# Chen001117/mappo

Measured on AMD Instinct MI355X. Metric: agent-steps/sec (collect+GAE+PPO), MPE simple_spread 3-agent, higher is better.
Workload: dtype f32; 1 GPU; BASELINE configs[1]: MPE simple_spread shape, 3 agents, obs 18 / share_obs 54 / Discrete(5), n_rollout_threads=1024 in total (strong scaling: 1024 on rank 0 of 1), episode_length=25, MLP policy (mappo), ppo_epoch=10, num_mini_batch=1, lr 7e-4, env=synthetic; n_rollout_threads_global=1024, n_rollout_threads_rank0=1024, episode_length=25, num_agents=3, ppo_epoch=10, num_mini_batch=1, parallelism=dp1, rccl_ranks=0, exact_minibatch_order=False, hip_graph=True

## Files before the change

### include/mappo_hip.h

```cpp
#ifndef MAPPO_HIP_H
#define MAPPO_HIP_H

#include <stdint.h>

#ifdef __cplusplus
extern "C" {
#endif

typedef void *mappo_stream_t;

#define MAPPO_OK 0
#define MAPPO_EINVAL (-1)
#define MAPPO_ELAUNCH (-2)
#define MAPPO_ENOTIMPL (-3)

#define MAPPO_HIDDEN 64
#define MAPPO_MAX_IN_DIM 512
#define MAPPO_MAX_ACTIONS 32
#define MAPPO_MAX_LAYER_N 2

const char *mappo_last_error(void);
int mappo_abi_version(void);

typedef struct {
// ... 19 lines not shown
                         float *rnn_dst, float *rnn_critic_dst, int32_t H, mappo_stream_t stream);

int mappo_insert_smac(const float *obs, const float *share_obs, const float *avail, const float *rewards, int64_t rew_stride_n,
                      int64_t rew_stride_m, const uint8_t *dones, int64_t done_stride_n, int64_t done_stride_m,
                      const uint8_t *bad_transition, const float *rnn_states, const float *rnn_states_critic, float *obs_dst,
                      float *share_dst, float *avail_dst, float *rew_dst, float *mask_dst, float *bad_mask_dst,
                      float *active_mask_dst, float *rnn_dst, float *rnn_critic_dst, int32_t N, int32_t M, int32_t D, int32_t S,
                      int32_t A, int32_t H, mappo_stream_t stream);

int mappo_recurrent_rows(const int64_t *perm, int32_t n_epochs, int64_t data_chunks, int32_t L, int32_t T, int32_t R,
                         int32_t num_mini_batch, int32_t *rows, int32_t *h0_rows, mappo_stream_t stream);

int mappo_copy_batch(int32_t count, float *const *dst, const float *const *src, const int64_t *n_floats, mappo_stream_t stream);

int mappo_gae_scan(const float *rewards , float *value_preds ,
                   const float *next_value , const float *masks ,
                   const float *bad_masks , float *returns ,
                   const float *vn_state , int32_t T, int32_t R, float gamma,
                   float gae_lambda, int32_t use_gae, int32_t use_proper_time_limits,
                   mappo_stream_t stream);

int64_t mappo_adv_workspace_bytes(int64_t n);
int mappo_adv_moments(const float *returns , const float *value_preds ,
                      const float *active_masks , const float *vn_state ,
                      float *adv , double *moments , void *workspace,
                      int64_t n, mappo_stream_t stream);
int mappo_adv_normalize(float *adv , const double *moments , int64_t n,
                        mappo_stream_t stream);

int64_t mappo_moments_workspace_bytes(int64_t B);
int mappo_minibatch_moments(const float *returns, const float *active_masks, const int32_t *rows,
                            int64_t B, double *mb_moments , void *workspace,
                            mappo_stream_t stream);
int mappo_valuenorm_update(float *vn_state , const double *mb_moments ,
                           double beta, mappo_stream_t stream);
int mappo_valuenorm_update_n(float *vn_state , const double *mb_moments , double beta, int32_t n,
                             float *states_out , mappo_stream_t stream);

typedef struct {
  float clip_param, entropy_coef, value_loss_coef, huber_delta;
  int32_t use_huber_loss, use_clipped_value_loss, use_policy_active_masks, use_value_active_masks,
      use_valuenorm;
  int32_t accumulate_partials;
} mappo_ppo_cfg;

int64_t mappo_ppo_loss_workspace_bytes(int64_t B);
int mappo_ppo_loss_fwd_bwd(const float *logits ,
                           const float *values , const int32_t *rows ,
                           const float *avail , const float *actions,
                           const float *old_logp, const float *adv, const float *active,
                           const float *v_old, const float *returns ,
                           const float *vn_state ,
                           const double *mb_moments ,
                           float *dlogits , float *dvalues , double *stats ,
                           void *workspace, const mappo_ppo_cfg *cfg , int64_t B, int32_t A,
                           mappo_stream_t stream);

int mappo_mlp_forward(const float *params, const mappo_net_desc *desc , const float *x ,
                      const int32_t *rows , int64_t B, float *out ,
                      mappo_stream_t stream);
int mappo_actor_act(const float *params, const mappo_net_desc *desc , const float *obs,
                    const float *avail , int64_t B, int32_t deterministic,
                    uint64_t seed, uint64_t counter, const uint64_t *counter_dev ,
                    float *actions , float *logp , mappo_stream_t stream);
int mappo_rollout_step(const float *actor_params, const mappo_net_desc *actor_desc , const float *critic_params,
                       const mappo_net_desc *critic_desc , const float *obs, int64_t obs_stride_n,
                       int64_t obs_stride_m, const float *share_obs, int64_t share_stride_n, int64_t share_stride_m,
                       int32_t M, int64_t B, const float *avail , int32_t deterministic, uint64_t seed,
                       uint64_t counter, const uint64_t *counter_dev, float *actions , float *logp ,
                       float *values , float *obs_dst , float *share_dst, const float *rewards,
                       int64_t rew_stride_n, int64_t rew_stride_m, const uint8_t *dones, int64_t done_stride_n,
                       int64_t done_stride_m, float *rew_dst, float *mask_dst, int32_t centralized, mappo_stream_t stream);
int mappo_actor_act_md(const float *params, const mappo_net_desc *desc , const float *obs, const float *avail ,
                       const int32_t *head_dims , int32_t n_heads, int64_t B, int32_t deterministic, uint64_t seed,
                       uint64_t counter, const uint64_t *counter_dev, float *actions , float *logp ,
                       mappo_stream_t stream);
int mappo_rollout_step_md(const float *actor_params, const mappo_net_desc *actor_desc , const float *critic_params,
                          const mappo_net_desc *critic_desc , const float *obs, int64_t obs_stride_n, int64_t obs_stride_m,
                          const float *share_obs, int64_t share_stride_n, int64_t share_stride_m, int32_t M, int64_t B,
                          const float *avail , const int32_t *head_dims , int32_t n_heads, int32_t deterministic,
                          uint64_t seed, uint64_t counter, const uint64_t *counter_dev, float *actions , float *logp ,
                          float *values , float *obs_dst , float *share_dst, const float *rewards,
                          int64_t rew_stride_n, int64_t rew_stride_m, const uint8_t *dones, int64_t done_stride_n, int64_t done_stride_m,
                          float *rew_dst, float *mask_dst, int32_t centralized, mappo_stream_t stream);
int mappo_rollout_episode(const float *actor_params, const mappo_net_desc *actor_desc , const float *critic_params,
                          const mappo_net_desc *critic_desc , int32_t T, int32_t N, int32_t M, const float *env_obs,
                          int64_t obs_stride_t, int64_t obs_stride_n, int64_t obs_stride_m, const float *rewards,
                          int64_t rew_stride_t, int64_t rew_stride_n, int64_t rew_stride_m, const uint8_t *dones,
                          int64_t done_stride_t, int64_t done_stride_n, int64_t done_stride_m, int32_t deterministic,
                          uint64_t seed, uint64_t counter, const uint64_t *counter_dev, float *obs_buf, float *share_buf,
                          float *rew_buf, float *mask_buf, float *actions , float *logp ,
                          float *values , float *next_values , int32_t centralized, mappo_stream_t stream);
int mappo_rollout_episode_uses_lds(int32_t layer_N);
int32_t mappo_mlp_backward_slabs(int64_t B);
int mappo_mlp_backward(const float *params, const mappo_net_desc *desc , const float *x,
                       const int32_t *rows, int64_t B, const float *dout ,
                       float *slabs, int64_t slab_stride, int64_t slab_col0,
                       float *wide_ws ,
                       mappo_stream_t stream);
#define MAPPO_WIDE_LAYOUT_FEATURE_MAJOR 0
#define MAPPO_WIDE_LAYOUT_BLOCKED 1
#define MAPPO_PRODUCER_MLP_BACKWARD 0
#define MAPPO_PRODUCER_ACTOR_UPDATE 1
#define MAPPO_PRODUCER_CRITIC_UPDATE 2
#define MAPPO_PRODUCER_TRUNK_BACKWARD 3
int64_t mappo_wide_workspace_floats(int64_t B);
int32_t mappo_wide_l1_slabs(int64_t B);
int32_t mappo_wide_layout(const mappo_net_desc *desc , int32_t producer );
int mappo_wide_l1_backward(const float *params, const mappo_net_desc *desc , const float *x, const int32_t *rows,
                           int64_t B, const float *wide_ws, float *slabs, int64_t slab_stride, int64_t slab_col0,
                           int32_t layout ,
                           mappo_stream_t stream);

int64_t mappo_update_partials_bytes(void);
int mappo_actor_update(const float *params, const mappo_net_desc *desc , const float *obs,
                       const int32_t *rows, int64_t B, const float *avail , const float *actions,
                       const float *old_logp, const float *adv, const float *active,
                       const double *mb_moments , const mappo_ppo_cfg *cfg , float *slabs,
                       int64_t slab_stride, int64_t slab_col0, double *partials, float *wide_ws ,
                       int32_t n_blocks ,
                       mappo_stream_t stream);
int mappo_critic_update(const float *params, const mappo_net_desc *desc , const float *share_obs,
                        const int32_t *rows, int64_t B, const float *v_old, const float *returns,
                        const float *active, const float *vn_state ,
                        const double *mb_moments , const mappo_ppo_cfg *cfg , float *slabs,
                        int64_t slab_stride, int64_t slab_col0, double *partials, float *wide_ws ,
                        int32_t n_blocks, mappo_stream_t stream);
int32_t mappo_dual_update_slabs(const mappo_net_desc *actor_desc , const mappo_net_desc *critic_desc , int64_t B);
int mappo_actor_critic_update(const float *actor_params, const mappo_net_desc *actor_desc , const float *obs,
                              const float *critic_params, const mappo_net_desc *critic_desc , const float *share_obs,
                              const int32_t *rows, int64_t B, const float *avail, const float *actions, const float *old_logp,
                              const float *adv, const float *active, const float *v_old, const float *returns,
                              const float *vn_state, const double *mb_moments, const mappo_ppo_cfg *cfg , float *slabs,
                              int64_t slab_stride, int64_t actor_col0, int64_t critic_col0, double *actor_partials,
                              double *critic_partials, mappo_stream_t stream);
int mappo_actor_update_md(const float *params, const mappo_net_desc *desc , const float *obs, const int32_t *rows, int64_t B,
                          const float *avail , const int32_t *head_dims , int32_t n_heads, const float *actions ,
                          const float *old_logp , const float *adv, const float *active, const double *mb_moments ,
                          const mappo_ppo_cfg *cfg , float *slabs, int64_t slab_stride, int64_t slab_col0, double *partials,
                          float *wide_ws , int32_t n_blocks, mappo_stream_t stream);
int mappo_actor_critic_update_md(const float *actor_params, const mappo_net_desc *actor_desc , const float *obs,
                                 const float *critic_params, const mappo_net_desc *critic_desc , const float *share_obs,
                                 const int32_t *rows, int64_t B, const float *avail , const int32_t *head_dims ,
                                 int32_t n_heads, const float *actions, const float *old_logp, const float *adv, const float *active,
                                 const float *v_old, const float *returns, const float *vn_state, const double *mb_moments,
                                 const mappo_ppo_cfg *cfg , float *slabs, int64_t slab_stride, int64_t actor_col0,
                                 int64_t critic_col0, double *actor_partials, double *critic_partials, mappo_stream_t stream);
int mappo_update_stats(const double *actor_partials, int32_t n_actor ,
                       const double *critic_partials, int32_t n_critic, const double *mb_moments,
                       const mappo_ppo_cfg *cfg , double *stats ,
                       double *acc ,
                       mappo_stream_t stream);

int mappo_mlp_features(const float *params, const mappo_net_desc *desc , const float *x, const int32_t *rows,
                       int64_t B, float *featT , mappo_stream_t stream);
int mappo_gru_forward(const float *params, const mappo_net_desc *desc , const float *featT, const float *h0,
                      const int32_t *h0_rows , const float *masks, const int32_t *rows ,
                      int32_t L, int32_t Nc, float *h_last ,
                      int32_t head_mode, float *out, const float *avail , int32_t deterministic,
                      uint64_t seed, uint64_t counter, const uint64_t *counter_dev, float *actions, float *logp,
                      mappo_stream_t stream);
int mappo_gru_step_dual(const float *actor_params, const mappo_net_desc *actor_desc , const float *actor_featT ,
                        const float *actor_h0 , float *actor_h_last, const float *critic_params,
                        const mappo_net_desc *critic_desc , const float *critic_featT, const float *critic_h0,
                        float *critic_h_last, const float *masks , int32_t Nc, const float *avail ,
                        int32_t deterministic, uint64_t seed, uint64_t counter, const uint64_t *counter_dev, float *actions,
                        float *logp, float *values, mappo_stream_t stream);
int mappo_recurrent_step_dual(const float *actor_params, const mappo_net_desc *actor_desc, const float *obs,
                              const float *actor_h0, float *actor_h_last, const float *critic_params,
                              const mappo_net_desc *critic_desc, const float *share_obs, const float *critic_h0,
                              float *critic_h_last, const float *masks, int32_t Nc, const float *avail, int32_t deterministic,
                              uint64_t seed, uint64_t counter, const uint64_t *counter_dev, float *actions, float *logp,
                              float *values, mappo_stream_t stream);
typedef struct mappo_smac_slot {
  float *obs, *share_obs, *available_actions , *rewards , *masks, *bad_masks, *active_masks, *rnn_states,
        *rnn_states_critic;
} mappo_smac_slot;
int mappo_recurrent_rollout_step(const float *actor_params, const mappo_net_desc *actor_desc , const float *critic_params,
                                 const mappo_net_desc *critic_desc , const float *obs, const float *share_obs, const float *avail,
                                 const float *rewards, int64_t rew_stride_n, int64_t rew_stride_m, const uint8_t *dones,
                                 int64_t done_stride_n, int64_t done_stride_m, const uint8_t *bad_transition ,
                                 const float *actor_h, const float *critic_h, float *actor_h_next, float *critic_h_next, int32_t N, int32_t M,
                                 int32_t deterministic, uint64_t seed, uint64_t counter, const uint64_t *counter_dev, float *actions,
                                 float *logp, float *values, const mappo_smac_slot *dst , mappo_stream_t stream);
int mappo_mlp_features_dual(const float *params_a, const mappo_net_desc *desc_a , const float *x_a, float *featT_a,
                            const float *params_c, const mappo_net_desc *desc_c , const float *x_c, float *featT_c,
                            int64_t B, mappo_stream_t stream);
int mappo_trunk_backward(const float *params, const mappo_net_desc *desc , const float *x, const int32_t *rows,
                         int64_t B, const float *dxT , float *slabs, int64_t slab_stride, int64_t slab_col0,
                         float *wide_ws , mappo_stream_t stream);

int64_t mappo_gru16_scratch_floats(int32_t L, int32_t Nc);
int64_t mappo_gru16_blocked_floats(int32_t L, int32_t Nc);
int32_t mappo_gru16_slabs(int32_t L, int32_t Nc);
int mappo_mlp_features_seq(const float *params, const mappo_net_desc *desc , const float *x, const int32_t *rows ,
                           int32_t L, int32_t Nc, float *out_blocked, mappo_stream_t stream);
int mappo_gru16_forward_loss(const float *params, const mappo_net_desc *desc , const float *x, int32_t x_blocked, const float *h0,
                             const int32_t *h0_rows , const float *masks, const int32_t *rows ,
                             int32_t L, int32_t Nc, int32_t head , const float *avail, const float *actions,
                             const float *old_logp, const float *adv, const float *active, const float *v_old, const float *returns,
                             const float *vn_state, const double *mb_moments, const mappo_ppo_cfg *cfg , float *scratch,
                             float *slabs, int64_t slab_stride, int64_t slab_col0, double *partials, mappo_stream_t stream);
int mappo_gru16_backward(const float *params, const mappo_net_desc *desc , const float *masks, const int32_t *rows, int32_t L,
                         int32_t Nc, float *scratch, float *dxT ,
                         mappo_stream_t stream);
int mappo_gru16_wgrad(const mappo_net_desc *desc , const float *x, int32_t x_blocked, const float *scratch, int32_t L, int32_t Nc,
                      float *slabs, int64_t slab_stride, int64_t slab_col0, mappo_stream_t stream);
int mappo_trunk_backward_seq(const float *params, const mappo_net_desc *desc , const float *x, const int32_t *rows, int32_t L,
                             int32_t Nc, const float *dx_blocked, float *slabs, int64_t slab_stride, int64_t slab_col0,
                             float *wide_ws ,
                             mappo_stream_t stream);

int64_t mappo_optim_workspace_bytes(int64_t P);
int mappo_slab_reduce(const float *slabs, int32_t n_slabs, int64_t slab_stride, int64_t P,
                      float *grad , mappo_stream_t stream);
int mappo_clip_adam(float *params, const float *grad, float *exp_avg, float *exp_avg_sq,
                    const int64_t *seg_bounds , int32_t n_seg,
                    const float *opt_hyper, int32_t *opt_step, float *grad_norms,
                    double *norm_acc , void *workspace,
                    mappo_stream_t stream);
int mappo_reduce_clip_adam(const float *slabs, int32_t n_slabs, int64_t slab_stride, float *params, float *grad ,
                           float *exp_avg, float *exp_avg_sq, const int64_t *seg_bounds , int32_t n_seg,
                           const float *opt_hyper, int32_t *opt_step, float *grad_norms, double *norm_acc ,
                           void *workspace, mappo_stream_t stream);

int mappo_mpe_spread_reset(double *agent_pos, double *agent_vel, double *landmark_pos, int32_t *tstep, int64_t *episode, float *obs,
                           int32_t N, int32_t M, int32_t L, uint64_t seed, mappo_stream_t stream);
int mappo_mpe_spread_step(double *agent_pos, double *agent_vel, double *landmark_pos, int32_t *tstep, int64_t *episode,
                          const float *actions, int32_t action_mode, float *obs, float *rewards, uint8_t *dones, int32_t N, int32_t M,
                          int32_t L, int32_t episode_length, uint64_t seed, mappo_stream_t stream);
int mappo_rollout_episode_spread(const float *actor_params, const mappo_net_desc *actor_desc , const float *critic_params,
                                 const mappo_net_desc *critic_desc , int32_t T, int32_t N, int32_t M, int32_t L,
                                 int32_t env_episode_length, uint64_t env_seed, double *agent_pos, double *agent_vel,
                                 double *landmark_pos, int32_t *tstep, int64_t *episode, int32_t deterministic, uint64_t seed,
                                 uint64_t counter, const uint64_t *counter_dev, float *obs_buf, float *share_buf, float *rew_buf,
                                 float *mask_buf, float *actions , float *logp , float *values ,
                                 float *next_values , int32_t centralized, mappo_stream_t stream);

int mappo_mpe_reference_reset(double *agent_pos, double *agent_vel, double *landmark_pos, int32_t *goal, int32_t *tstep,
                              int64_t *episode, float *obs, int32_t N, uint64_t seed, mappo_stream_t stream);
int mappo_mpe_reference_step(double *agent_pos, double *agent_vel, double *landmark_pos, int32_t *goal, int32_t *tstep,
                             int64_t *episode, const float *actions, int32_t action_mode, float *obs, float *rewards, uint8_t *dones,
                             int32_t N, int32_t episode_length, uint64_t seed, mappo_stream_t stream);
int mappo_rollout_episode_reference(const float *actor_params, const mappo_net_desc *actor_desc , const float *critic_params,
                                    const mappo_net_desc *critic_desc , const int32_t *head_dims ,
                                    int32_t n_heads, int32_t T, int32_t N, int32_t env_episode_length, uint64_t env_seed,
                                    double *agent_pos, double *agent_vel, double *landmark_pos, int32_t *goal, int32_t *tstep,
                                    int64_t *episode, int32_t deterministic, uint64_t seed, uint64_t counter,
                                    const uint64_t *counter_dev, float *obs_buf, float *share_buf, float *rew_buf, float *mask_buf,
                                    float *actions , float *logp , float *values ,
                                    float *next_values , int32_t centralized, mappo_stream_t stream);

int mappo_mpe_comm_reset(double *listener_pos, double *listener_vel, double *landmark_pos, int32_t *goal, int32_t *symbol,
                         int32_t *tstep, int64_t *episode, float *obs_speaker, float *obs_listener, int32_t N, uint64_t seed,
                         mappo_stream_t stream);
int mappo_mpe_comm_step(double *listener_pos, double *listener_vel, double *landmark_pos, int32_t *goal, int32_t *symbol,
                        int32_t *tstep, int64_t *episode, const float *actions_speaker, const float *actions_listener,
                        int32_t action_mode, float *obs_speaker, float *obs_listener, float *rewards, uint8_t *dones, int32_t N,
                        int32_t episode_length, uint64_t seed, mappo_stream_t stream);
typedef struct mappo_comm_agent {
  const float *actor_params, *critic_params;
  mappo_net_desc actor_desc, critic_desc;
  uint64_t seed;
  const uint64_t *counter_dev;
  float *obs_buf, *share_buf, *rew_buf, *mask_buf, *actions, *logp, *values, *next_values;
} mappo_comm_agent;
int mappo_rollout_episode_comm(const mappo_comm_agent *speaker , const mappo_comm_agent *listener , int32_t T,
                               int32_t N, int32_t env_episode_length, uint64_t env_seed, double *listener_pos, double *listener_vel,
                               double *landmark_pos, int32_t *goal, int32_t *symbol, int32_t *tstep, int64_t *episode,
                               int32_t deterministic, uint64_t counter, int32_t centralized,
                               mappo_stream_t stream);

int mappo_mpe_adversary_reset(double *agent_pos, double *agent_vel, double *landmark_pos, int32_t *goal, int32_t *tstep,
                              int64_t *episode, float *obs_adversary, float *obs_good1, float *obs_good2, int32_t N,
                              int32_t num_agents, uint64_t seed, mappo_stream_t stream);
int mappo_mpe_adversary_step(double *agent_pos, double *agent_vel, double *landmark_pos, int32_t *goal, int32_t *tstep,
                             int64_t *episode, const float *actions, int32_t action_mode, float *obs_adversary, float *obs_good1,
                             float *obs_good2, float *rewards, uint8_t *dones, int32_t N, int32_t num_agents,
                             int32_t episode_length, uint64_t seed, mappo_stream_t stream);
int mappo_rollout_episode_adversary(const mappo_comm_agent *agents , double *agent_pos, double *agent_vel,
                                    double *landmark_pos, int32_t *goal, int32_t *tstep, int64_t *episode, int32_t T, int32_t N,
                                    int32_t env_episode_length, uint64_t env_seed, int32_t deterministic, uint64_t counter,
                                    int32_t centralized, mappo_stream_t stream);

int mappo_synth_smac_pool(float *obs, float *share_obs, float *avail, float *rewards, uint8_t *dead, uint8_t *dones, int32_t P,
                          int32_t N, int32_t M, int32_t D, int32_t S, int32_t A, float p_death, float p_term, uint64_t seed,
                          uint64_t *counter_dev , mappo_stream_t stream);
int mappo_synth_smac_step(float *obs, float *share_obs, float *avail, float *rewards, uint8_t *dead, uint8_t *dones,
                          int32_t N, int32_t M, int32_t D, int32_t S, int32_t A, float p_death, float p_term,
                          uint64_t seed, uint64_t *counter_dev , mappo_stream_t stream);

#define MAPPO_PROF_GAE 0
#define MAPPO_PROF_PPO_LOSS 1
#define MAPPO_PROF_MLP_FWD 2
#define MAPPO_PROF_MLP_BWD 3
#define MAPPO_PROF_SLAB_REDUCE 4
#define MAPPO_PROF_ADAM 5
#define MAPPO_PROF_ACT 6
#define MAPPO_PROF_COUNT 8
int mappo_profile_arm(int32_t kernel_id, void *ev_start , void *ev_stop );

int mappo_selftest_mfma(const float *A , const float *Bm , float *D ,
                        mappo_stream_t stream);

#ifdef __cplusplus
}
// ... 3 lines not shown
```

### mappo_amd/_lib.py

```python
import ctypes as C
import os

import torch

_HERE = os.path.dirname(os.path.abspath(__file__))
LIB_PATH = os.environ.get("MAPPO_HIP_LIB") or os.path.join(_HERE, "libmappo_hip.so")

HIDDEN = 64
MAX_ACTIONS = 32
MAX_LAYER_N = 2


class NetDesc(C.Structure):
    _fields_ = [("in_dim", C.c_int32), ("hidden", C.c_int32), ("out_dim", C.c_int32), ("layer_N", C.c_int32),
                ("use_relu", C.c_int32), ("use_feature_norm", C.c_int32), ("recurrent", C.c_int32)]


class PpoCfg(C.Structure):
    _fields_ = [("clip_param", C.c_float), ("entropy_coef", C.c_float), ("value_loss_coef", C.c_float),
                ("huber_delta", C.c_float), ("use_huber_loss", C.c_int32), ("use_clipped_value_loss", C.c_int32),
                ("use_policy_active_masks", C.c_int32), ("use_value_active_masks", C.c_int32),
                ("use_valuenorm", C.c_int32), ("accumulate_partials", C.c_int32)]


class SmacSlot(C.Structure):
    _fields_ = [(n, C.c_void_p) for n in ("obs", "share_obs", "available_actions", "rewards", "masks", "bad_masks", "active_masks",
                                          "rnn_states", "rnn_states_critic")]


class CommAgent(C.Structure):
    _fields_ = ([("actor_params", C.c_void_p), ("critic_params", C.c_void_p), ("actor_desc", NetDesc), ("critic_desc", NetDesc),
                 ("seed", C.c_uint64), ("counter_dev", C.c_void_p)] +
                [(n, C.c_void_p) for n in ("obs_buf", "share_buf", "rew_buf", "mask_buf", "actions", "logp", "values", "next_values")])


_P, _I32, _I64, _F, _D, _U64 = C.c_void_p, C.c_int32, C.c_int64, C.c_float, C.c_double, C.c_uint64

SIGNATURES = {
    "mappo_last_error": (C.c_char_p, []),
    "mappo_abi_version": (C.c_int, []),
    "mappo_net_param_count": (_I64, [C.POINTER(NetDesc)]),
    "mappo_insert_mpe": (C.c_int, [_P, _I64, _I64, _P, _I64, _I64, _P, _I64, _I64, _P, _P, _P, _P, _I32, _I32, _I32, _I32, _P]),
    "mappo_insert_mpe_rnn": (C.c_int, [_P, _I64, _I64, _P, _I64, _I64, _P, _I64, _I64, _P, _P, _P, _P, _I32, _I32, _I32, _I32, _P, _P, _P, _P,
                                       _I32, _P]),
    "mappo_insert_smac": (C.c_int, [_P, _P, _P, _P, _I64, _I64, _P, _I64, _I64, _P, _P, _P] + [_P] * 9 + [_I32] * 6 + [_P]),
    "mappo_recurrent_rows": (C.c_int, [_P, _I32, _I64, _I32, _I32, _I32, _I32, _P, _P, _P]),
    "mappo_copy_batch": (C.c_int, [_I32, C.POINTER(C.c_void_p), C.POINTER(C.c_void_p), C.POINTER(_I64), _P]),
    "mappo_gae_scan": (C.c_int, [_P, _P, _P, _P, _P, _P, _P, _I32, _I32, _F, _F, _I32, _I32, _P]),
    "mappo_adv_workspace_bytes": (_I64, [_I64]),
    "mappo_adv_moments": (C.c_int, [_P, _P, _P, _P, _P, _P, _P, _I64, _P]),
    "mappo_adv_normalize": (C.c_int, [_P, _P, _I64, _P]),
    "mappo_moments_workspace_bytes": (_I64, [_I64]),
    "mappo_minibatch_moments": (C.c_int, [_P, _P, _P, _I64, _P, _P, _P]),
    "mappo_valuenorm_update": (C.c_int, [_P, _P, _D, _P]),
    "mappo_valuenorm_update_n": (C.c_int, [_P, _P, _D, _I32, _P, _P]),
    "mappo_ppo_loss_workspace_bytes": (_I64, [_I64]),
    "mappo_ppo_loss_fwd_bwd": (C.c_int, [_P] * 16 + [C.POINTER(PpoCfg), _I64, _I32, _P]),
    "mappo_mlp_forward": (C.c_int, [_P, C.POINTER(NetDesc), _P, _P, _I64, _P, _P]),
    "mappo_actor_act": (C.c_int, [_P, C.POINTER(NetDesc), _P, _P, _I64, _I32, _U64, _U64, _P, _P, _P, _P]),
    "mappo_rollout_step": (C.c_int, [_P, C.POINTER(NetDesc), _P, C.POINTER(NetDesc), _P, _I64, _I64, _P, _I64, _I64, _I32, _I64, _P, _I32,
                                     _U64, _U64, _P, _P, _P, _P, _P, _P, _P, _I64, _I64, _P, _I64, _I64, _P, _P, _I32, _P]),
    "mappo_actor_act_md": (C.c_int, [_P, C.POINTER(NetDesc), _P, _P, C.POINTER(_I32), _I32, _I64, _I32, _U64, _U64, _P, _P, _P, _P]),
    "mappo_rollout_step_md": (C.c_int, [_P, C.POINTER(NetDesc), _P, C.POINTER(NetDesc), _P, _I64, _I64, _P, _I64, _I64, _I32, _I64, _P,
                                        C.POINTER(_I32), _I32, _I32, _U64, _U64, _P, _P, _P, _P, _P, _P, _P, _I64, _I64, _P, _I64, _I64, _P, _P,
                                        _I32, _P]),
    "mappo_rollout_episode": (C.c_int, [_P, C.POINTER(NetDesc), _P, C.POINTER(NetDesc), _I32, _I32, _I32, _P, _I64, _I64, _I64, _P, _I64,
                                        _I64, _I64, _P, _I64, _I64, _I64, _I32, _U64, _U64, _P, _P, _P, _P, _P, _P, _P, _P, _P, _I32, _P]),
    "mappo_rollout_episode_uses_lds": (C.c_int, [_I32]),
    "mappo_mlp_backward_slabs": (_I32, [_I64]),
    "mappo_mlp_backward": (C.c_int, [_P, C.POINTER(NetDesc), _P, _P, _I64, _P, _P, _I64, _I64, _P, _P]),
    "mappo_wide_workspace_floats": (_I64, [_I64]),
    "mappo_wide_l1_slabs": (_I32, [_I64]),
    "mappo_wide_layout": (_I32, [C.POINTER(NetDesc), _I32]),
    "mappo_wide_l1_backward": (C.c_int, [_P, C.POINTER(NetDesc), _P, _P, _I64, _P, _P, _I64, _I64, _I32, _P]),
    "mappo_update_partials_bytes": (_I64, []),
    "mappo_actor_update": (C.c_int, [_P, C.POINTER(NetDesc), _P, _P, _I64, _P, _P, _P, _P, _P, _P, C.POINTER(PpoCfg), _P, _I64,
                                     _I64, _P, _P, _I32, _P]),
    "mappo_critic_update": (C.c_int, [_P, C.POINTER(NetDesc), _P, _P, _I64, _P, _P, _P, _P, _P, C.POINTER(PpoCfg), _P, _I64,
                                      _I64, _P, _P, _I32, _P]),
    "mappo_dual_update_slabs": (_I32, [C.POINTER(NetDesc), C.POINTER(NetDesc), _I64]),
    "mappo_actor_critic_update": (C.c_int, [_P, C.POINTER(NetDesc), _P, _P, C.POINTER(NetDesc), _P, _P, _I64, _P, _P, _P, _P, _P, _P, _P, _P, _P,
                                            C.POINTER(PpoCfg), _P, _I64, _I64, _I64, _P, _P, _P]),
    "mappo_actor_update_md": (C.c_int, [_P, C.POINTER(NetDesc), _P, _P, _I64, _P, C.POINTER(_I32), _I32, _P, _P, _P, _P, _P, C.POINTER(PpoCfg),
                                        _P, _I64, _I64, _P, _P, _I32, _P]),
    "mappo_actor_critic_update_md": (C.c_int, [_P, C.POINTER(NetDesc), _P, _P, C.POINTER(NetDesc), _P, _P, _I64, _P, C.POINTER(_I32), _I32,
                                               _P, _P, _P, _P, _P, _P, _P, _P, C.POINTER(PpoCfg), _P, _I64, _I64, _I64, _P, _P, _P]),
    "mappo_update_stats": (C.c_int, [_P, _I32, _P, _I32, _P, C.POINTER(PpoCfg), _P, _P, _P]),
    "mappo_mlp_features": (C.c_int, [_P, C.POINTER(NetDesc), _P, _P, _I64, _P, _P]),
    "mappo_gru_forward": (C.c_int, [_P, C.POINTER(NetDesc), _P, _P, _P, _P, _P, _I32, _I32, _P, _I32, _P, _P, _I32, _U64, _U64,
                                    _P, _P, _P, _P]),
    "mappo_gru_step_dual": (C.c_int, [_P, C.POINTER(NetDesc), _P, _P, _P, _P, C.POINTER(NetDesc), _P, _P, _P, _P, _I32, _P, _I32, _U64, _U64,
                                      _P, _P, _P, _P, _P]),
    "mappo_recurrent_step_dual": (C.c_int, [_P, C.POINTER(NetDesc), _P, _P, _P, _P, C.POINTER(NetDesc), _P, _P, _P, _P, _I32, _P, _I32, _U64, _U64,
                                      _P, _P, _P, _P, _P]),
    "mappo_gru16_scratch_floats": (_I64, [_I32, _I32]),
    "mappo_gru16_blocked_floats": (_I64, [_I32, _I32]),
    "mappo_gru16_slabs": (_I32, [_I32, _I32]),
    "mappo_mlp_features_seq": (C.c_int, [_P, C.POINTER(NetDesc), _P, _P, _I32, _I32, _P, _P]),
    "mappo_gru16_forward_loss": (C.c_int, [_P, C.POINTER(NetDesc), _P, _I32, _P, _P, _P, _P, _I32, _I32, _I32] + [_P] * 9 +
                                 [C.POINTER(PpoCfg), _P, _P, _I64, _I64, _P, _P]),
    "mappo_gru16_backward": (C.c_int, [_P, C.POINTER(NetDesc), _P, _P, _I32, _I32, _P, _P, _P]),
    "mappo_gru16_wgrad": (C.c_int, [C.POINTER(NetDesc), _P, _I32, _P, _I32, _I32, _P, _I64, _I64, _P]),
    "mappo_trunk_backward_seq": (C.c_int, [_P, C.POINTER(NetDesc), _P, _P, _I32, _I32, _P, _P, _I64, _I64, _P, _P]),
    "mappo_recurrent_rollout_step": (C.c_int, [_P, C.POINTER(NetDesc), _P, C.POINTER(NetDesc), _P, _P, _P, _P, _I64, _I64, _P, _I64, _I64, _P,
                                               _P, _P, _P, _P, _I32, _I32, _I32, _U64, _U64, _P, _P, _P, _P, C.POINTER(SmacSlot), _P]),
    "mappo_mlp_features_dual": (C.c_int, [_P, C.POINTER(NetDesc), _P, _P, _P, C.POINTER(NetDesc), _P, _P, _I64, _P]),
    "mappo_trunk_backward": (C.c_int, [_P, C.POINTER(NetDesc), _P, _P, _I64, _P, _P, _I64, _I64, _P, _P]),
    "mappo_optim_workspace_bytes": (_I64, [_I64]),
    "mappo_slab_reduce": (C.c_int, [_P, _I32, _I64, _I64, _P, _P]),
    "mappo_clip_adam": (C.c_int, [_P, _P, _P, _P, C.POINTER(_I64), _I32, _P, _P, _P, _P, _P, _P]),
    "mappo_reduce_clip_adam": (C.c_int, [_P, _I32, _I64, _P, _P, _P, _P, C.POINTER(_I64), _I32, _P, _P, _P, _P, _P, _P]),
    "mappo_mpe_spread_reset": (C.c_int, [_P, _P, _P, _P, _P, _P, _I32, _I32, _I32, _U64, _P]),
    "mappo_synth_smac_pool": (C.c_int, [_P, _P, _P, _P, _P, _P, _I32, _I32, _I32, _I32, _I32, _I32, C.c_float, C.c_float, _U64, _P, _P]),
    "mappo_synth_smac_step": (C.c_int, [_P, _P, _P, _P, _P, _P, _I32, _I32, _I32, _I32, _I32, C.c_float, C.c_float, _U64, _P, _P]),
    "mappo_mpe_spread_step": (C.c_int, [_P, _P, _P, _P, _P, _P, _I32, _P, _P, _P, _I32, _I32, _I32, _I32, _U64, _P]),
    "mappo_rollout_episode_spread": (C.c_int, [_P, C.POINTER(NetDesc), _P, C.POINTER(NetDesc), _I32, _I32, _I32, _I32, _I32, _U64, _P, _P, _P, _P,
                                               _P, _I32, _U64, _U64, _P, _P, _P, _P, _P, _P, _P, _P, _P, _I32, _P]),
    "mappo_mpe_reference_reset": (C.c_int, [_P, _P, _P, _P, _P, _P, _P, _I32, _U64, _P]),
    "mappo_mpe_reference_step": (C.c_int, [_P, _P, _P, _P, _P, _P, _P, _I32, _P, _P, _P, _I32, _I32, _U64, _P]),
    "mappo_rollout_episode_reference": (C.c_int, [_P, C.POINTER(NetDesc), _P, C.POINTER(NetDesc), C.POINTER(_I32), _I32, _I32, _I32, _I32, _U64,
                                                  _P, _P, _P, _P, _P, _P, _I32, _U64, _U64, _P, _P, _P, _P, _P, _P, _P, _P, _P, _I32, _P]),
    "mappo_mpe_comm_reset": (C.c_int, [_P, _P, _P, _P, _P, _P, _P, _P, _P, _I32, _U64, _P]),
    "mappo_mpe_comm_step": (C.c_int, [_P, _P, _P, _P, _P, _P, _P, _P, _P, _I32, _P, _P, _P, _P, _I32, _I32, _U64, _P]),
    "mappo_rollout_episode_comm": (C.c_int, [C.POINTER(CommAgent), C.POINTER(CommAgent), _I32, _I32, _I32, _U64, _P, _P, _P, _P, _P, _P, _P,
                                             _I32, _U64, _I32, _P]),
    "mappo_mpe_adversary_reset": (C.c_int, [_P, _P, _P, _P, _P, _P, _P, _P, _P, _I32, _I32, _U64, _P]),
    "mappo_mpe_adversary_step": (C.c_int, [_P, _P, _P, _P, _P, _P, _P, _I32, _P, _P, _P, _P, _P, _I32, _I32, _I32, _U64, _P]),
    "mappo_rollout_episode_adversary": (C.c_int, [C.POINTER(CommAgent), _P, _P, _P, _P, _P, _P, _I32, _I32, _I32, _U64, _I32, _U64, _I32, _P]),
    "mappo_profile_arm": (C.c_int, [_I32, _P, _P]),
    "mappo_selftest_mfma": (C.c_int, [_P, _P, _P, _P]),
}

_lib = None


class MappoHipError(RuntimeError):
    pass


def load():
    global _lib
    if _lib is not None:
        return _lib
    if not os.path.exists(LIB_PATH):
        raise MappoHipError(f"{LIB_PATH} is missing — build it with `python -m mappo_amd.build` "
                            "(hipcc --offload-arch=gfx950).  There is no CPU fallback for the MAPPO hot path.")
    lib = C.CDLL(LIB_PATH)
    for name, (res, args) in SIGNATURES.items():
        fn = getattr(lib, name)
        fn.restype, fn.argtypes = res, args
    _lib = lib
    return lib


def check(rc, what):
    if rc != 0:
        msg = load().mappo_last_error().decode("utf-8", "replace")
        raise MappoHipError(f"{what} failed (code {rc}): {msg}")
```

### mappo_amd/algorithms/r_mappo/r_mappo.py

```python
import numpy as np
import os
import torch

from mappo_amd import ops
from mappo_amd.utils.util import to_device_f32
from mappo_amd.utils.valuenorm import ValueNorm


class R_MAPPO():
    def __init__(self, args, policy, device=torch.device("cuda"), dist_group=None):
        self.device = torch.device(device)
        self.tpdv = dict(dtype=torch.float32, device=self.device)
        self.policy = policy
        self.args = args

        self.clip_param = args.clip_param
        self.ppo_epoch = args.ppo_epoch
        self.num_mini_batch = args.num_mini_batch
        self.data_chunk_length = args.data_chunk_length
        self.value_loss_coef = args.value_loss_coef
        self.entropy_coef = args.entropy_coef
        self.max_grad_norm = args.max_grad_norm
        self.huber_delta = args.huber_delta

        self._use_recurrent_policy = args.use_recurrent_policy
        self._use_naive_recurrent = args.use_naive_recurrent_policy
        self._use_max_grad_norm = args.use_max_grad_norm
        self._use_clipped_value_loss = args.use_clipped_value_loss
        self._use_huber_loss = args.use_huber_loss
        self._use_popart = args.use_popart
        self._use_valuenorm = args.use_valuenorm
        self._use_value_active_masks = args.use_value_active_masks
        self._use_policy_active_masks = args.use_policy_active_masks
        self._exact_order = bool(getattr(args, "exact_minibatch_order", False))
        self._fused = not bool(getattr(args, "unfused_update", False))
        self._use_graph = bool(getattr(args, "use_hip_graph", True))
        self._concurrent_update = bool(getattr(args, "concurrent_update", False))
        self._graphs = {}
        self._dp_graphs = {}
        self._graph_buffers = {}

        assert (self._use_popart and self._use_valuenorm) == False, \
            "self._use_popart and self._use_valuenorm can not be set True simultaneously"
        if self._use_popart:
            raise NotImplementedError("use_popart: PopArt.update raises in the reference itself (SURVEY.md §8c)")
        self.value_normalizer = ValueNorm(1, device=self.device) if self._use_valuenorm else None

        self._cfg = ops.ppo_cfg(args)
        self._cfg_acc = ops.ppo_cfg(args, accumulate_partials=True)
        self._dual_update = bool(getattr(args, "dual_update", True)) and os.environ.get("MAPPO_DUAL_UPDATE", "1") != "0"
        self._epochs = None
        self._dist = dist_group
        if getattr(policy.actor, "head_dims", None):
            if dist_group is not None:
                raise NotImplementedError("MultiDiscrete action space under the data-parallel trainer: the multi-head update is built for "
                                          "single-process training only")
            if not self._fused:
                raise NotImplementedError("unfused_update with a MultiDiscrete action space: the loss of several heads exists in the fused "
                                          "update kernels only")
        if dist_group is not None:
            from mappo_amd.distributed import sampling_seed
            policy.actor._seed = sampling_seed(int(getattr(args, "seed", 1)), dist_group.rank)
        f64 = dict(dtype=torch.float64, device=self.device)
        self._mb_moments = torch.zeros(4, **f64)
        self._adv_moments = torch.zeros(3, **f64)
        self._stats = torch.zeros(6, **f64)
        self._zbuf = torch.zeros(8 + 2 * 1024, **f64)
        self._acc = self._zbuf[:6]
        self._pa, self._pc = self._zbuf[8:8 + 1024], self._zbuf[8 + 1024:]
        self._ws = {}
        self._training = False

    def _buf(self, name, shape, dtype=torch.float32, zero=False):
        key = (name, tuple(shape), dtype)
        t = self._ws.get(key)
        if t is None:
            t = (torch.zeros if zero else torch.empty)(shape, dtype=dtype, device=self.device)
            self._ws[key] = t
        return t

    def _bytes(self, name, nbytes):
        return self._buf(name, (int(nbytes),), torch.uint8)

    def _update(self, src, rows, B, update_actor=True, moments_ready=False, part="all"):
        pol = self.policy
        A = pol.actor.n_actions
        lib = ops._lib.load()
        vn_state = self.value_normalizer.state if self._use_valuenorm else None
        n_slabs = ops.mlp_backward_slabs(B)
        P = pol.n_flat
        if part != "optim":
            self._slab_rows = n_slabs
            slabs = self._update_kernels(src, rows, B, update_actor, moments_ready, vn_state, n_slabs, P)
            n_slabs = self._slab_rows
        else:
            slabs = self._buf("slabs", (n_slabs, P))
        if update_actor != self._actor_enabled and part != "kernels":
            pol.opt_hyper[0, 7] = 1.0 if update_actor else 0.0
            self._actor_enabled = update_actor
        if self._dist is None:
            ops.reduce_clip_adam(slabs, n_slabs, P, pol.flat_params, pol.flat_grad, pol.exp_avg, pol.exp_avg_sq, pol.seg_bounds,
                                 pol.opt_hyper, pol.opt_step, pol.grad_norms, pol.opt_workspace, norm_acc=self._acc[4:])
            return
        if part != "optim":
            ops.slab_reduce(slabs, n_slabs, P, P, pol.flat_grad)
        if part != "kernels":
            self._dist.all_reduce_sum_(pol.flat_grad)
            ops.clip_adam(pol.flat_params, pol.flat_grad, pol.exp_avg, pol.exp_avg_sq, pol.seg_bounds, pol.opt_hyper,
                          pol.opt_step, pol.grad_norms, pol.opt_workspace, norm_acc=self._acc[4:])

    def _moments(self, src, rows, B, vn_state):
        lib = ops._lib.load()
        ops.minibatch_moments(src["returns"], src["active"], rows, B, self._mb_moments,
                              self._bytes("mom_ws", lib.mappo_moments_workspace_bytes(B)))
        if self._dist is not None:
            self._dist.all_reduce_sum_(self._mb_moments)
        ep = self._epochs
        if ep is not None and self._use_valuenorm:
            ops.valuenorm_update_n(vn_state, self._mb_moments, self.value_normalizer.beta, ep["n"], ep["states"])

    def _update_kernels(self, src, rows, B, update_actor, moments_ready, vn_state, n_slabs, P):
        pol = self.policy
        A = pol.actor.n_actions
        lib = ops._lib.load()
        ep = self._epochs
        if not moments_ready:
            self._moments(src, rows, B, vn_state)
        cfg = self._cfg
        if ep is not None:
            cfg = self._cfg_acc
            if self._use_valuenorm:
                vn_state = ep["states"][ep["e"]]
        elif self._use_valuenorm:
            ops.valuenorm_update(vn_state, self._mb_moments, self.value_normalizer.beta)
        hd = pol.actor.head_dims
        slabs = self._buf("slabs", (n_slabs, P), zero=True)
        if not update_actor and not self._actor_slabs_clean:
            slabs[:, :pol.seg_bounds[1]].zero_()
        self._actor_slabs_clean = not update_actor
        if self._fused:
            pa, pc = self._pa, self._pc
            na, nc = (0, 0)
            if update_actor and self._concurrent_update and not hd:
                na, nc = self._split_grid(n_slabs, pol.actor.desc.in_dim, pol.critic.desc.in_dim, B)
            if na:
                cur = torch.cuda.current_stream()
                if self._side_stream is None:
                    self._side_stream = torch.cuda.Stream(device=self.device)
                side = self._side_stream
                side.wait_stream(cur)
                with torch.cuda.stream(side):
                    ops.actor_update(pol.actor.flat, pol.actor.desc, src["obs"], rows, B, src["avail"], src["actions"],
                                     src["old_logp"], src["adv"], src["active"], self._mb_moments, cfg, slabs, P, 0, pa, na)
                ops.critic_update(pol.critic.flat, pol.critic.desc, src["share_obs"], rows, B, src["v_old"], src["returns"],
                                  src["active"], vn_state, self._mb_moments, cfg, slabs, P, pol.seg_bounds[1], pc, nc)
                cur.wait_stream(side)
                n_pa, n_pc = na, nc
            elif hd and update_actor and self._dual_update and pol.can_dual_update():
                ops.actor_critic_update_md(pol.actor.flat, pol.actor.desc, src["obs"], pol.critic.flat, pol.critic.desc, src["share_obs"],
                                           rows, B, hd, src["actions"], src["old_logp"], src["adv"], src["active"], src["v_old"],
                                           src["returns"], vn_state, self._mb_moments, cfg, slabs, P, 0, pol.seg_bounds[1], pa, pc)
                n_pa = n_pc = ops.dual_update_slabs(pol.actor.desc, pol.critic.desc, B)
                self._slab_rows = n_pa
            elif update_actor and self._dual_update and pol.can_dual_update():
                ops.actor_critic_update(pol.actor.flat, pol.actor.desc, src["obs"], pol.critic.flat, pol.critic.desc, src["share_obs"],
                                        rows, B, src["avail"], src["actions"], src["old_logp"], src["adv"], src["active"], src["v_old"],
                                        src["returns"], vn_state, self._mb_moments, cfg, slabs, P, 0, pol.seg_bounds[1], pa, pc)
                n_pa = n_pc = ops.dual_update_slabs(pol.actor.desc, pol.critic.desc, B)
                self._slab_rows = n_pa
            else:
                if update_actor and hd:
                    ops.actor_update_md(pol.actor.flat, pol.actor.desc, src["obs"], rows, B, hd, src["actions"], src["old_logp"],
                                        src["adv"], src["active"], self._mb_moments, cfg, slabs, P, 0, pa)
                elif update_actor:
                    ops.actor_update(pol.actor.flat, pol.actor.desc, src["obs"], rows, B, src["avail"], src["actions"],
                                     src["old_logp"], src["adv"], src["active"], self._mb_moments, cfg, slabs, P, 0, pa)
                ops.critic_update(pol.critic.flat, pol.critic.desc, src["share_obs"], rows, B, src["v_old"], src["returns"],
                                  src["active"], vn_state, self._mb_moments, cfg, slabs, P, pol.seg_bounds[1], pc)
                n_pa = n_pc = n_slabs
            if ep is None:
                ops.update_stats(pa if update_actor else None, n_pa, pc, n_pc, self._mb_moments, self._cfg, self._stats, self._acc)

        else:
            logits = self._buf("logits", (B, A))
            values = self._buf("values", (B,))
            ops.mlp_forward(pol.actor.flat, pol.actor.desc, src["obs"], rows, B, logits)
            ops.mlp_forward(pol.critic.flat, pol.critic.desc, src["share_obs"], rows, B, values)
            dlogits = self._buf("dlogits", (B, A))
            dvalues = self._buf("dvalues", (B,))
            ops.ppo_loss_fwd_bwd(logits, values, rows, src["avail"], src["actions"], src["old_logp"], src["adv"],
                                 src["active"], src["v_old"], src["returns"], vn_state, self._mb_moments, dlogits, dvalues,
                                 self._stats, self._cfg, self._bytes("loss_ws", lib.mappo_ppo_loss_workspace_bytes(B)))
            self._acc[:4].add_(self._stats[:4])
            if update_actor:
                ops.mlp_backward(pol.actor.flat, pol.actor.desc, src["obs"], rows, B, dlogits, slabs, P, 0)
            ops.mlp_backward(pol.critic.flat, pol.critic.desc, src["share_obs"], rows, B, dvalues, slabs, P, pol.seg_bounds[1])
        return slabs

    _actor_slabs_clean = True
    _actor_enabled = True
    _side_stream = None

    @staticmethod
    def _split_grid(n_slabs, d_actor, d_critic, B):
        if n_slabs < 256 or d_actor > 64 or d_critic > 64:
            return 0, 0
        tiles = (B + 31) // 32
        cost = lambda d: 1.0 + 0.25 * (d > 32)
        best = None
        for na in range(96, 161, 4):
            nc = 256 - na
            t = max(-(-tiles // (4 * na)) * cost(d_actor), -(-tiles // (4 * nc)) * cost(d_critic))
            if best is None or t < best[0]:
                best = (t, na, nc)
        return best[1], best[2]

    def _buffer_sources(self, buffer, adv):
        T = buffer.episode_length
        R = buffer.n_rollout_threads * buffer.num_agents
        S = T * R
        flat = lambda a: a[:T].view(S, -1)
        return dict(obs=flat(buffer.obs), share_obs=flat(buffer.share_obs),
                    avail=flat(buffer.available_actions) if buffer.available_actions is not None else None,
                    actions=buffer.actions.view(S, -1).squeeze(-1), old_logp=buffer.action_log_probs.view(S, -1).squeeze(-1), adv=adv,
                    active=buffer.active_masks[:T].view(S), v_old=buffer.value_preds[:T].view(S),
                    returns=buffer.returns[:T].view(S)), S

    @torch.no_grad()
    def train(self, buffer, update_actor=True, after_update=False):
        self._sync_actor_mode(update_actor)
        if self._use_recurrent_policy or self._use_naive_recurrent:
            from mappo_amd.recurrent import train_recurrent
            static = buffer.perm_device != "cpu"
            body = lambda: (train_recurrent(self, buffer, update_actor), buffer.after_update() if after_update else None)
        else:
            static = self.num_mini_batch == 1 and not self._exact_order
            body = lambda: self._train_body(buffer, update_actor, after_update)
        if not (self._use_graph and static and self._dist is None):
            body()
            return self._finish_train_info()
        key = (self._buffer_key(buffer), bool(update_actor), bool(after_update))
        state = self._graphs.get(key)
        if state is None:
            body()
            self._graphs[key] = "warm"
        else:
            if state == "warm":
                torch.cuda.synchronize()
                g = torch.cuda.CUDAGraph()
                with torch.cuda.graph(g):
                    body()
                self._graphs[key] = state = g
            state.replay()
        return self._finish_train_info()

    def _buffer_key(self, buffer):
        k = id(buffer)
        held = self._graph_buffers.setdefault(k, buffer)
        assert held is buffer
        return k

    def _sync_actor_mode(self, update_actor):
        if update_actor != self._actor_enabled:
            self.policy.opt_hyper[0, 7] = 1.0 if update_actor else 0.0
            self._actor_enabled = update_actor
        if not update_actor and not self._actor_slabs_clean:
            for (name, _, _), t in self._ws.items():
                if name == "slabs" or name.startswith("slabs_rec/"):
                    t[:, :self.policy.seg_bounds[1]].zero_()
        self._actor_slabs_clean = not update_actor

    def _train_body(self, buffer, update_actor, after_update):
        T = buffer.episode_length
        S = T * buffer.n_rollout_threads * buffer.num_agents
        adv = self.compute_advantages(buffer)
        src, _ = self._buffer_sources(buffer, adv)
        self._zbuf.zero_()
        whole = self.num_mini_batch == 1 and not self._exact_order
        dp_graph = self._dist is not None and self._use_graph and whole and self._fused and self._dist.world_is_gpu
        key = (self._buffer_key(buffer), bool(update_actor))
        self._epochs = None
        if whole and self._fused and (self._dist is None or dp_graph) and not self._concurrent_update \
                and os.environ.get("MAPPO_EPOCH_BATCH", "1") != "0":
            self._epochs = dict(n=self.ppo_epoch, e=0, states=self._buf("vn_states", (self.ppo_epoch, 3)))
        if dp_graph:
            vn_state = self.value_normalizer.state if self._use_valuenorm else None
            self._moments(src, None, S, vn_state)
        for epoch in range(self.ppo_epoch):
            if self._epochs is not None:
                self._epochs["e"] = epoch
            if whole:
                batches = [(None, S)]
            else:
                batches = [(rows, rows.numel()) for rows in buffer.feed_forward_rows(self.num_mini_batch)]
            for rows, B in batches:
                if dp_graph:
                    gkey = key + (epoch,)
                    st = self._dp_graphs.get(gkey)
                    if st is None and self._dp_graphs.get(key) == "warm":
                        st = "warm"
                    if st == "warm":
                        torch.cuda.synchronize()
                        try:
                            g = torch.cuda.CUDAGraph()
                            with torch.cuda.graph(g, capture_error_mode="thread_local"):
                                self._update(src, rows, B, update_actor, moments_ready=True, part="kernels")
                            self._dp_graphs[gkey] = st = g
                        except Exception as e:
                            import warnings
                            warnings.warn(f"hipGraph capture of the data-parallel update segment failed ({e}); launching eagerly")
                            torch.cuda.synchronize()
                            self._dp_graphs[gkey] = st = "off"
                    if st == "off":
                        st = None
                    if st is None:
                        self._update(src, rows, B, update_actor, moments_ready=True, part="kernels")
                    else:
                        st.replay()
                    self._update(src, rows, B, update_actor, moments_ready=True, part="optim")
                else:
                    self._update(src, rows, B, update_actor, moments_ready=whole and epoch > 0)
        if self._epochs is not None:
            n_rows = ops.dual_update_slabs(self.policy.actor.desc, self.policy.critic.desc, S) if (update_actor and self._dual_update and self.policy.can_dual_update()) \
                else ops.mlp_backward_slabs(S)
            ops.update_stats(self._pa if update_actor else None, n_rows, self._pc, n_rows, self._mb_moments, self._cfg, self._stats,
                             self._acc)
            self._epochs = None
        if dp_graph and self._dp_graphs.get(key) is None:
            self._dp_graphs[key] = "warm"
        if after_update:
            buffer.after_update()

    def compute_advantages(self, buffer):
        T = buffer.episode_length
        S = T * buffer.n_rollout_threads * buffer.num_agents
        adv = self._buf("adv", (S,))
        lib = ops._lib.load()
        vn_state = self.value_normalizer.state if self._use_valuenorm else None
        ops.adv_moments(buffer.returns[:T].view(S), buffer.value_preds[:T].view(S), buffer.active_masks[:T].view(S), vn_state,
                        adv, self._adv_moments, self._bytes("adv_ws", lib.mappo_adv_workspace_bytes(S)))
        if self._dist is not None:
            self._dist.all_reduce_sum_(self._adv_moments)
        ops.adv_normalize(adv, self._adv_moments)
        return adv

    def _finish_train_info(self):
        num_updates = self.ppo_epoch * self.num_mini_batch
        if self._dist is not None:
            self._dist.all_reduce_sum_(self._acc[:4])
        acc = (self._acc / max(num_updates, 1)).cpu().numpy()
        return dict(value_loss=float(acc[0]), policy_loss=float(acc[1]), dist_entropy=float(acc[2]),
                    actor_grad_norm=float(acc[4]), critic_grad_norm=float(acc[5]), ratio=float(acc[3]))

    @torch.no_grad()
    def ppo_update(self, sample, update_actor=True):
        if self._use_recurrent_policy or self._use_naive_recurrent:
            from mappo_amd.recurrent import ppo_update_recurrent
            return ppo_update_recurrent(self, sample, update_actor)
        (share_obs, obs, rnn_a, rnn_c, actions, v_old, ret, masks, active, old_logp, adv, avail) = sample
        d = lambda x: to_device_f32(x, self.device)
        B = np.shape(obs)[0] if not torch.is_tensor(obs) else obs.shape[0]
        src = dict(obs=d(obs), share_obs=d(share_obs), avail=d(avail) if avail is not None else None,
                   actions=d(actions).view(B, -1).squeeze(-1), old_logp=d(old_logp).view(B, -1).squeeze(-1), adv=d(adv).view(B),
                   active=d(active).view(B),
                   v_old=d(v_old).view(B), returns=d(ret).view(B))
        self._acc.zero_()
        self._update(src, None, B, update_actor)
        a = self._acc.cpu().numpy()
        return a[0], a[5], a[1], a[2], a[4], a[3]

    @torch.no_grad()
    def cal_value_loss(self, values, value_preds_batch, return_batch, active_masks_batch):
        d = lambda x: to_device_f32(x, self.device)
        values, value_preds_batch, return_batch, active_masks_batch = d(values), d(value_preds_batch), d(return_batch), d(active_masks_batch)
        clipped = value_preds_batch + (values - value_preds_batch).clamp(-self.clip_param, self.clip_param)
        if self._use_valuenorm:
            self.value_normalizer.update(return_batch)
            tgt = self.value_normalizer.normalize(return_batch)
        else:
            tgt = return_batch
        e_c, e_o = tgt - clipped, tgt - values

        def loss(e):
            if self._use_huber_loss:
                dl = self.huber_delta
                return torch.where(e.abs() <= dl, e * e / 2, dl * (e.abs() - dl / 2))
            return e * e / 2
        l = torch.max(loss(e_o), loss(e_c)) if self._use_clipped_value_loss else loss(e_o)
        if self._use_value_active_masks:
            return (l * active_masks_batch).sum() / active_masks_batch.sum()
        return l.mean()

    def prep_training(self):
        self._training = True

    def prep_rollout(self):
        self._training = False
```

### mappo_amd/config.py

```python
import argparse


def get_config():
    p = argparse.ArgumentParser(description="mappo_amd", formatter_class=argparse.RawDescriptionHelpFormatter)
    off = dict(action="store_false", default=True)
    on = dict(action="store_true", default=False)
    p.add_argument("--algorithm_name", type=str, default="mappo", choices=["rmappo", "mappo"])
    p.add_argument("--experiment_name", type=str, default="check")
    p.add_argument("--seed", type=int, default=1)
    p.add_argument("--cuda", **off)
    p.add_argument("--cuda_deterministic", **off)
    p.add_argument("--n_training_threads", type=int, default=1)
    p.add_argument("--n_rollout_threads", type=int, default=32)
    p.add_argument("--n_eval_rollout_threads", type=int, default=1)
    p.add_argument("--n_render_rollout_threads", type=int, default=1)
    p.add_argument("--num_env_steps", type=int, default=10e6)
    p.add_argument("--user_name", type=str, default="marl")
    p.add_argument("--use_wandb", **off)
    p.add_argument("--env_name", type=str, default="StarCraft2")
    p.add_argument("--use_obs_instead_of_state", **on)
    p.add_argument("--episode_length", type=int, default=200)
    p.add_argument("--share_policy", **off)
    p.add_argument("--use_centralized_V", **off)
    p.add_argument("--stacked_frames", type=int, default=1)
    p.add_argument("--use_stacked_frames", **on)
    p.add_argument("--hidden_size", type=int, default=64)
    p.add_argument("--layer_N", type=int, default=1)
    p.add_argument("--use_ReLU", **off)
    p.add_argument("--use_popart", **on)
    p.add_argument("--use_valuenorm", **off)
    p.add_argument("--use_feature_normalization", **off)
    p.add_argument("--use_orthogonal", **off)
    p.add_argument("--gain", type=float, default=0.01)
    p.add_argument("--use_naive_recurrent_policy", **on)
    p.add_argument("--use_recurrent_policy", **off)
    p.add_argument("--recurrent_N", type=int, default=1)
    p.add_argument("--data_chunk_length", type=int, default=10)
    p.add_argument("--lr", type=float, default=5e-4)
    p.add_argument("--critic_lr", type=float, default=5e-4)
    p.add_argument("--opti_eps", type=float, default=1e-5)
    p.add_argument("--weight_decay", type=float, default=0)
    p.add_argument("--ppo_epoch", type=int, default=15)
    p.add_argument("--use_clipped_value_loss", **off)
    p.add_argument("--clip_param", type=float, default=0.2)
    p.add_argument("--num_mini_batch", type=int, default=1)
    p.add_argument("--entropy_coef", type=float, default=0.01)
    p.add_argument("--value_loss_coef", type=float, default=1)
    p.add_argument("--use_max_grad_norm", **off)
    p.add_argument("--max_grad_norm", type=float, default=10.0)
    p.add_argument("--use_gae", **off)
    p.add_argument("--gamma", type=float, default=0.99)
    p.add_argument("--gae_lambda", type=float, default=0.95)
    p.add_argument("--use_proper_time_limits", **on)
    p.add_argument("--use_huber_loss", **off)
    p.add_argument("--use_value_active_masks", **off)
    p.add_argument("--use_policy_active_masks", **off)
    p.add_argument("--huber_delta", type=float, default=10.0)
    p.add_argument("--use_linear_lr_decay", **on)
    p.add_argument("--save_interval", type=int, default=1)
    p.add_argument("--log_interval", type=int, default=5)
    p.add_argument("--use_eval", **on)
    p.add_argument("--eval_interval", type=int, default=25)
    p.add_argument("--eval_episodes", type=int, default=32)
    p.add_argument("--save_gifs", **on)
    p.add_argument("--use_render", **on)
    p.add_argument("--render_episodes", type=int, default=5)
    p.add_argument("--ifi", type=float, default=0.1)
    p.add_argument("--model_dir", type=str, default=None)
    p.add_argument("--exact_minibatch_order", **on,
                   help="with num_mini_batch == 1 the minibatch is the whole buffer and its permutation only reorders "
                        "the terms of sums; by default the kernels then stream the buffer in place. Set to gather by "
                        "the random permutation anyway (what the reference's generator does).")
    p.add_argument("--unfused_update", **on,
                   help="run each PPO update as separate forward / fused-loss / backward launches (the standalone C-ABI ops) "
                        "instead of the one-launch-per-network update kernels; same results")
    p.add_argument("--use_hip_graph", **off,
                   help="by default the launch-bound inner loops (PPO updates; rollout with a graph-safe env) are captured "
                        "into hipGraphs after one eager pass; pass the flag to always launch eagerly")
    p.add_argument("--host_staging", **off,
                   help="by default the NumPy output of a CPU vec-env goes through pinned double-buffered staging blocks "
                        "(mappo_amd/utils/host_staging.py) and feeds the same one-launch rollout step as a device env; pass the "
                        "flag to upload with plain torch copies")
    p.add_argument("--fuse_rollout_step", **off,
                   help="by default an MLP policy's rollout step (insert of the previous env output + get_actions + get_values) "
                        "is ONE kernel launch (mappo_rollout_step); pass the flag to use the separate insert / actor / critic launches")
    p.add_argument("--fuse_rollout_episode", **off,
                   help="by default, with an env that hands out a whole episode up front (SyntheticMPEEnv.episode_block) and a "
                        "narrow MLP policy, the rollout episode (T x get_actions, T + 1 x get_values, every insert) is ONE kernel "
                        "launch (mappo_rollout_episode); with the GPU-resident simple_spread env (SimpleSpreadVecEnv.episode_state) the env "
                        "steps run inside that launch too (mappo_rollout_episode_spread), and so they do with the GPU-resident simple_reference env "
                        "and its MultiDiscrete (5, 10) policy (SimpleReferenceVecEnv, mappo_rollout_episode_reference); pass the flag to run "
                        "the stepwise loop")
    p.add_argument("--dual_update", **off,
                   help="by default the actor's and the critic's fused update run in ONE launch, half the CUs each "
                        "(mappo_actor_critic_update); pass the flag to launch them one after the other")
    p.add_argument("--concurrent_update", **on,
                   help="launch the actor and critic update kernels side by side on a split grid (two streams); measured "
                        "slower than back-to-back full-size launches on MI355X, kept for experiments")
    p.add_argument("--perm_device", type=str, default="cuda", choices=["cuda", "cpu"],
                   help="where torch.randperm runs; 'cpu' reproduces the reference's permutation stream bit-exactly")
    return p


def mpe_defaults(parser):
    parser.add_argument("--scenario_name", type=str, default="simple_spread",
                        help="MPE scenario; GPU-resident envs exist for simple_spread, simple_reference, simple_speaker_listener "
                             "(num_agents 2, share_policy False) and simple_adversary (num_agents 3, share_policy False): mappo_amd.envs")
    parser.add_argument("--num_landmarks", type=int, default=3)
    parser.add_argument("--num_agents", type=int, default=2)
    return parser


def apply_algorithm_name(all_args):
    if all_args.algorithm_name == "rmappo":
        all_args.use_recurrent_policy, all_args.use_naive_recurrent_policy = True, False
    elif all_args.algorithm_name == "mappo":
        all_args.use_recurrent_policy, all_args.use_naive_recurrent_policy = False, False
    else:
        raise NotImplementedError(all_args.algorithm_name)
    return all_args
```

### mappo_amd/csrc/error.hip

```cpp
#include "common.h"
#include <string.h>

static thread_local char g_err[512] = "";

void mappo_set_error(const char *fmt, ...) {
  va_list ap;
  va_start(ap, fmt);
  vsnprintf(g_err, sizeof(g_err), fmt, ap);
  va_end(ap);
}

extern "C" const char *mappo_last_error(void) { return g_err; }
extern "C" int mappo_abi_version(void) { return 7; }

ProfSlot g_prof[MAPPO_PROF_COUNT] = {};

extern "C" int mappo_profile_arm(int32_t kernel_id, void *ev_start, void *ev_stop) {
  MAPPO_REQUIRE(kernel_id >= 0 && kernel_id < MAPPO_PROF_COUNT, "profile_arm: kernel_id %d", kernel_id);
  g_prof[kernel_id].start = (hipEvent_t)ev_start;
  g_prof[kernel_id].stop = (hipEvent_t)ev_stop;
  return MAPPO_OK;
}
```

### mappo_amd/csrc/insert.hip

```cpp
#include "insert_core.h"

__global__ __launch_bounds__(256) void insert_mpe_kernel(InsertArgs p) { insert_mpe_body(p, blockIdx.x, gridDim.x); }

extern "C" int mappo_insert_mpe(const float *obs, int64_t obs_stride_n, int64_t obs_stride_m, const float *rewards,
                                int64_t rew_stride_n, int64_t rew_stride_m, const uint8_t *dones, int64_t done_stride_n,
                                int64_t done_stride_m, float *obs_dst, float *share_dst, float *rew_dst, float *mask_dst,
                                int32_t N, int32_t M, int32_t D, int32_t centralized, mappo_stream_t stream) {
  MAPPO_REQUIRE(obs && rewards && dones && obs_dst && share_dst && rew_dst && mask_dst && N > 0 && M > 0 && D > 0,
                "insert_mpe: bad arguments");
  InsertArgs a;
  a.obs = obs; a.obs_sn = obs_stride_n; a.obs_sm = obs_stride_m; a.rew = rewards; a.rew_sn = rew_stride_n; a.rew_sm = rew_stride_m;
  a.done = dones; a.done_sn = done_stride_n; a.done_sm = done_stride_m; a.obs_dst = obs_dst; a.share_dst = share_dst;
  a.rew_dst = rew_dst; a.mask_dst = mask_dst; a.N = N; a.M = M; a.D = D; a.centralized = centralized;
  const int64_t total = (int64_t)N * M * (centralized ? M * D : D);
  int64_t nb = (total + 255) / 256;
  if (nb > 2048) nb = 2048;
  hipLaunchKernelGGL(insert_mpe_kernel, dim3((unsigned)nb), dim3(256), 0, as_stream(stream), a);
  MAPPO_CHECK_LAUNCH("insert_mpe");
  return MAPPO_OK;
}

struct RnnInsert {
  const float *h_a, *h_c;
  float *dst_a, *dst_c;
  int H;
};
__global__ __launch_bounds__(256) void insert_mpe_rnn_kernel(InsertArgs p, RnnInsert r) {
  insert_mpe_body(p, blockIdx.x, gridDim.x);
  const int h4 = r.H >> 2;
  const int64_t total = (int64_t)p.N * p.M * h4;
  for (int64_t e = (int64_t)blockIdx.x * blockDim.x + threadIdx.x; e < total; e += (int64_t)gridDim.x * blockDim.x) {
    const int64_t nm = e / h4;
    const int n = (int)(nm / p.M), m = (int)(nm - (int64_t)n * p.M);
    const float keep = p.done[n * p.done_sn + m * p.done_sm] ? 0.f : 1.f;
    float4 a = reinterpret_cast<const float4 *>(r.h_a)[e], c = reinterpret_cast<const float4 *>(r.h_c)[e];
    a.x *= keep; a.y *= keep; a.z *= keep; a.w *= keep;
    c.x *= keep; c.y *= keep; c.z *= keep; c.w *= keep;
    reinterpret_cast<float4 *>(r.dst_a)[e] = a;
    reinterpret_cast<float4 *>(r.dst_c)[e] = c;
  }
}

extern "C" int mappo_insert_mpe_rnn(const float *obs, int64_t obs_stride_n, int64_t obs_stride_m, const float *rewards,
                                    int64_t rew_stride_n, int64_t rew_stride_m, const uint8_t *dones, int64_t done_stride_n,
                                    int64_t done_stride_m, float *obs_dst, float *share_dst, float *rew_dst, float *mask_dst,
                                    int32_t N, int32_t M, int32_t D, int32_t centralized, const float *rnn_states,
                                    const float *rnn_states_critic, float *rnn_dst, float *rnn_critic_dst, int32_t H,
                                    mappo_stream_t stream) {
  MAPPO_REQUIRE(obs && rewards && dones && obs_dst && share_dst && rew_dst && mask_dst && N > 0 && M > 0 && D > 0,
                "insert_mpe_rnn: bad arguments");
  MAPPO_REQUIRE(rnn_states && rnn_states_critic && rnn_dst && rnn_critic_dst && H > 0 && (H & 3) == 0, "insert_mpe_rnn: bad state arguments");
  MAPPO_REQUIRE(((((uintptr_t)rnn_states) | ((uintptr_t)rnn_states_critic) | ((uintptr_t)rnn_dst) | ((uintptr_t)rnn_critic_dst)) & 15) == 0,
                "insert_mpe_rnn: state arrays must be 16-byte aligned");
  InsertArgs a;
  a.obs = obs; a.obs_sn = obs_stride_n; a.obs_sm = obs_stride_m; a.rew = rewards; a.rew_sn = rew_stride_n; a.rew_sm = rew_stride_m;
  a.done = dones; a.done_sn = done_stride_n; a.done_sm = done_stride_m; a.obs_dst = obs_dst; a.share_dst = share_dst;
  a.rew_dst = rew_dst; a.mask_dst = mask_dst; a.N = N; a.M = M; a.D = D; a.centralized = centralized;
  RnnInsert r;
  r.h_a = rnn_states; r.h_c = rnn_states_critic; r.dst_a = rnn_dst; r.dst_c = rnn_critic_dst; r.H = H;
  const int64_t t1 = (int64_t)N * M * (centralized ? M * D : D), t2 = (int64_t)N * M * (H >> 2);
  int64_t nb = ((t1 > t2 ? t1 : t2) + 255) / 256;
  if (nb > 2048) nb = 2048;
  hipLaunchKernelGGL(insert_mpe_rnn_kernel, dim3((unsigned)nb), dim3(256), 0, as_stream(stream), a, r);
  MAPPO_CHECK_LAUNCH("insert_mpe_rnn");
  return MAPPO_OK;
}

__global__ __launch_bounds__(256) void insert_smac_kernel(SmacInsert p) { insert_smac_body(p, blockIdx.x, gridDim.x); }

extern "C" int mappo_insert_smac(const float *obs, const float *share_obs, const float *avail, const float *rewards, int64_t rew_stride_n,
                                 int64_t rew_stride_m, const uint8_t *dones, int64_t done_stride_n, int64_t done_stride_m,
                                 const uint8_t *bad_transition, const float *rnn_states, const float *rnn_states_critic, float *obs_dst,
                                 float *share_dst, float *avail_dst, float *rew_dst, float *mask_dst, float *bad_mask_dst,
                                 float *active_mask_dst, float *rnn_dst, float *rnn_critic_dst, int32_t N, int32_t M, int32_t D,
                                 int32_t S, int32_t A, int32_t H, mappo_stream_t stream) {
  MAPPO_REQUIRE(obs && share_obs && rewards && dones && obs_dst && share_dst && rew_dst && mask_dst && bad_mask_dst && active_mask_dst &&
                N > 0 && M > 0 && D > 0 && S > 0, "insert_smac: bad arguments");
  MAPPO_REQUIRE(!avail || (avail_dst && A > 0), "insert_smac: available_actions slot");
  if (rnn_states) {
    MAPPO_REQUIRE(rnn_states_critic && rnn_dst && rnn_critic_dst && H > 0 && (H & 3) == 0, "insert_smac: bad state arguments");
    MAPPO_REQUIRE(((((uintptr_t)rnn_states) | ((uintptr_t)rnn_states_critic) | ((uintptr_t)rnn_dst) | ((uintptr_t)rnn_critic_dst)) & 15) == 0,
                  "insert_smac: state arrays must be 16-byte aligned");
  }
  SmacInsert a;
  a.obs = obs; a.share = share_obs; a.avail = avail; a.rew = rewards; a.rew_sn = rew_stride_n; a.rew_sm = rew_stride_m;
  a.done = dones; a.done_sn = done_stride_n; a.done_sm = done_stride_m; a.bad = bad_transition; a.h_a = rnn_states; a.h_c = rnn_states_critic;
  a.obs_dst = obs_dst; a.share_dst = share_dst; a.avail_dst = avail_dst; a.rew_dst = rew_dst; a.mask_dst = mask_dst; a.bad_dst = bad_mask_dst;
  a.active_dst = active_mask_dst; a.ha_dst = rnn_dst; a.hc_dst = rnn_critic_dst; a.N = N; a.M = M; a.D = D; a.S = S; a.A = A; a.H = H;
  int64_t most = (int64_t)N * M * (D > S ? D : S);
  int64_t nb = (most + 255) / 256;
  if (nb > 2048) nb = 2048;
  hipLaunchKernelGGL(insert_smac_kernel, dim3((unsigned)nb), dim3(256), 0, as_stream(stream), a);
  MAPPO_CHECK_LAUNCH("insert_smac");
  return MAPPO_OK;
}

struct RecRows {
  const int64_t *perm;
  int32_t *rows, *h0;
  int64_t chunks;
  int E, L, T, R, nmb, mbs;
};
__global__ __launch_bounds__(256) void recurrent_rows_kernel(RecRows p) {
  const int64_t per_e = (int64_t)p.nmb * p.mbs, total = (int64_t)p.E * per_e * p.L;
  for (int64_t i = (int64_t)blockIdx.x * blockDim.x + threadIdx.x; i < total; i += (int64_t)gridDim.x * blockDim.x) {
    const int64_t j = i % p.mbs;
    const int l = (int)((i / p.mbs) % p.L);
    const int64_t ek = i / ((int64_t)p.mbs * p.L);
    const int64_t e = ek / p.nmb, k = ek - e * p.nmb;
    const int64_t c = p.perm[e * p.chunks + k * p.mbs + j];
    const int64_t q = c * p.L + l;
    const int32_t row = (int32_t)((q % p.T) * p.R + q / p.T);
    p.rows[i] = row;
    if (l == 0) p.h0[ek * p.mbs + j] = row;
  }
}

extern "C" int mappo_recurrent_rows(const int64_t *perm, int32_t n_epochs, int64_t data_chunks, int32_t L, int32_t T, int32_t R,
                                    int32_t num_mini_batch, int32_t *rows, int32_t *h0_rows, mappo_stream_t stream) {
  MAPPO_REQUIRE(perm && rows && h0_rows && n_epochs > 0 && data_chunks > 0 && L > 0 && T > 0 && R > 0 && num_mini_batch > 0,
                "recurrent_rows: bad arguments");
  MAPPO_REQUIRE(data_chunks / num_mini_batch > 0, "recurrent_rows: fewer chunks than minibatches");
  MAPPO_REQUIRE((int64_t)T * R < ((int64_t)1 << 31), "recurrent_rows: buffer rows exceed int32");
  RecRows a;
  a.perm = perm; a.rows = rows; a.h0 = h0_rows; a.chunks = data_chunks; a.E = n_epochs; a.L = L; a.T = T; a.R = R;
  a.nmb = num_mini_batch; a.mbs = (int)(data_chunks / num_mini_batch);
  const int64_t total = (int64_t)n_epochs * a.nmb * a.mbs * L;
  int64_t nb = (total + 255) / 256;
  if (nb > 4096) nb = 4096;
  hipLaunchKernelGGL(recurrent_rows_kernel, dim3((unsigned)nb), dim3(256), 0, as_stream(stream), a);
  MAPPO_CHECK_LAUNCH("recurrent_rows");
  return MAPPO_OK;
}

#define COPY_MAX 16
struct CopyBatch {
  float *dst[COPY_MAX];
  const float *src[COPY_MAX];
  int64_t n[COPY_MAX];
  int count;
};
__global__ __launch_bounds__(256) void copy_batch_kernel(CopyBatch c) {
  for (int j = 0; j < c.count; ++j) {
    const float *__restrict__ s = c.src[j];
    float *__restrict__ d = c.dst[j];
    const int64_t n = c.n[j];
    if (((((uintptr_t)s) | ((uintptr_t)d)) & 15) == 0) {
      const int64_t n4 = n >> 2;
      for (int64_t i = (int64_t)blockIdx.x * blockDim.x + threadIdx.x; i < n4; i += (int64_t)gridDim.x * blockDim.x)
        reinterpret_cast<float4 *>(d)[i] = reinterpret_cast<const float4 *>(s)[i];
      for (int64_t i = (n4 << 2) + (int64_t)blockIdx.x * blockDim.x + threadIdx.x; i < n; i += (int64_t)gridDim.x * blockDim.x) d[i] = s[i];
    } else {
      for (int64_t i = (int64_t)blockIdx.x * blockDim.x + threadIdx.x; i < n; i += (int64_t)gridDim.x * blockDim.x) d[i] = s[i];
    }
  }
}

extern "C" int mappo_copy_batch(int32_t count, float *const *dst, const float *const *src, const int64_t *n_floats,
                                mappo_stream_t stream) {
  MAPPO_REQUIRE(count >= 1 && count <= COPY_MAX && dst && src && n_floats, "copy_batch: bad arguments (count=%d)", count);
  CopyBatch c;
  c.count = count;
  int64_t total = 0;
  for (int j = 0; j < count; ++j) {
    MAPPO_REQUIRE(dst[j] && src[j] && n_floats[j] >= 0, "copy_batch: entry %d", j);
    c.dst[j] = dst[j]; c.src[j] = src[j]; c.n[j] = n_floats[j];
    total += n_floats[j];
  }
  int64_t nb = (total / 4 + 255) / 256;
  if (nb < 1) nb = 1;
  if (nb > 1024) nb = 1024;
  hipLaunchKernelGGL(copy_batch_kernel, dim3((unsigned)nb), dim3(256), 0, as_stream(stream), c);
  MAPPO_CHECK_LAUNCH("copy_batch");
  return MAPPO_OK;
}
```

### mappo_amd/csrc/insert_core.h

```cpp
#pragma once
#include "common.h"

struct InsertArgs {
  const float *obs;  int64_t obs_sn, obs_sm;
  const float *rew;  int64_t rew_sn, rew_sm;
  const uint8_t *done; int64_t done_sn, done_sm;
  float *obs_dst, *share_dst, *rew_dst, *mask_dst;
  int N, M, D, centralized;
};

__device__ __forceinline__ void insert_mpe_body(const InsertArgs &p, int bid, int nb) {
  const int S = p.centralized ? p.M * p.D : p.D;
  const int64_t total = (int64_t)p.N * p.M * S;
  for (int64_t e = (int64_t)bid * blockDim.x + threadIdx.x; e < total; e += (int64_t)nb * blockDim.x) {
    const int64_t nm = e / S;
    const int j = (int)(e - nm * S);
    const int n = (int)(nm / p.M), m = (int)(nm - (int64_t)n * p.M);
    const int ms = p.centralized ? j / p.D : m, d = p.centralized ? j - ms * p.D : j;
    const float v = p.obs[n * p.obs_sn + ms * p.obs_sm + d];
    p.share_dst[e] = v;
    if (!p.centralized || ms == m) p.obs_dst[nm * p.D + d] = v;
    if (j == 0) {
      p.rew_dst[nm] = p.rew[n * p.rew_sn + m * p.rew_sm];
      p.mask_dst[nm] = p.done[n * p.done_sn + m * p.done_sm] ? 0.f : 1.f;
    }
  }
}

template <int U, typename I>
__device__ __forceinline__ void insert_mpe_episode_run(const InsertArgs &p, int64_t obs_st, int64_t rew_st, int64_t done_st, int T,
                                                       int w, int nw) {
  const int S = p.centralized ? p.M * p.D : p.D;
  const int64_t R = (int64_t)p.N * p.M, RS = R * S, total = (int64_t)T * RS, nthr = (int64_t)nw * WAVE;
  for (int64_t e0 = (int64_t)w * WAVE + (threadIdx.x & (WAVE - 1)); e0 < total; e0 += U * nthr) {
    float v[U], rw[U];
    uint8_t dn[U];
    int64_t tn[U];
    int dd[U], jj[U];
#pragma unroll
    for (int u = 0; u < U; ++u) {
      const int64_t e = e0 + u * nthr;
      jj[u] = -1;
      if (e < total) {
        const I t = (I)e / (I)RS, rem = (I)e - t * (I)RS, nm = rem / (I)S;
        const int j = (int)(rem - nm * (I)S);
        const int n = (int)(nm / (I)p.M), m = (int)(nm - (I)n * (I)p.M);
        const int ms = p.centralized ? j / p.D : m, d = p.centralized ? j - ms * p.D : j;
        v[u] = p.obs[(int64_t)t * obs_st + n * p.obs_sn + ms * p.obs_sm + d];
        tn[u] = (int64_t)t * R + (int64_t)nm;
        dd[u] = (!p.centralized || ms == m) ? d : -1;
        jj[u] = j;
        if (j == 0) {
          rw[u] = p.rew[(int64_t)t * rew_st + n * p.rew_sn + m * p.rew_sm];
          dn[u] = p.done[(int64_t)t * done_st + n * p.done_sn + m * p.done_sm];
        }
      }
    }
    __builtin_amdgcn_sched_barrier(0);
    __builtin_amdgcn_s_waitcnt(0);
    __builtin_amdgcn_sched_barrier(0);
#pragma unroll
    for (int u = 0; u < U; ++u) {
      if (jj[u] < 0) continue;
      p.share_dst[e0 + u * nthr] = v[u];
      if (dd[u] >= 0) p.obs_dst[tn[u] * p.D + dd[u]] = v[u];
      if (jj[u] == 0) {
        p.rew_dst[tn[u]] = rw[u];
        p.mask_dst[tn[u]] = dn[u] != 0 ? 0.f : 1.f;
      }
    }
  }
}
template <int U>
__device__ __forceinline__ void insert_mpe_episode_body(const InsertArgs &p, int64_t obs_st, int64_t rew_st, int64_t done_st, int T,
                                                        int w, int nw) {
  const int64_t total = (int64_t)T * p.N * p.M * (p.centralized ? p.M * p.D : p.D);
  if (total <= (int64_t)UINT32_MAX) insert_mpe_episode_run<U, uint32_t>(p, obs_st, rew_st, done_st, T, w, nw);
  else insert_mpe_episode_run<U, int64_t>(p, obs_st, rew_st, done_st, T, w, nw);
}

struct SmacInsert {
  const float *obs, *share, *avail;
  const float *rew; int64_t rew_sn, rew_sm;
  const uint8_t *done; int64_t done_sn, done_sm;
  const uint8_t *bad;
  const float *h_a, *h_c;
  float *obs_dst, *share_dst, *avail_dst, *rew_dst, *mask_dst, *bad_dst, *active_dst, *ha_dst, *hc_dst;
  int N, M, D, S, A, H;
};
__device__ __forceinline__ bool env_done(const SmacInsert &p, int n) {
  bool all = true;
  for (int m = 0; m < p.M; ++m) all = all && p.done[n * p.done_sn + m * p.done_sm] != 0;
  return all;
}
__device__ __forceinline__ void insert_smac_body(const SmacInsert &p, int bid, int nb) {
  const int64_t tid = (int64_t)bid * blockDim.x + threadIdx.x, nthr = (int64_t)nb * blockDim.x;
  const int64_t R = (int64_t)p.N * p.M;
  for (int64_t e = tid; e < R * p.D; e += nthr) p.obs_dst[e] = p.obs[e];
  for (int64_t e = tid; e < R * p.S; e += nthr) p.share_dst[e] = p.share[e];
  if (p.avail)
    for (int64_t e = tid; e < R * p.A; e += nthr) p.avail_dst[e] = p.avail[e];
  for (int64_t e = tid; e < R; e += nthr) {
    const int n = (int)(e / p.M), m = (int)(e - (int64_t)n * p.M);
    const bool de = env_done(p, n), d = p.done[n * p.done_sn + m * p.done_sm] != 0;
    p.rew_dst[e] = p.rew[n * p.rew_sn + m * p.rew_sm];
    p.mask_dst[e] = de ? 0.f : 1.f;
    p.active_dst[e] = de ? 1.f : (d ? 0.f : 1.f);
    p.bad_dst[e] = (p.bad && p.bad[e]) ? 0.f : 1.f;
  }
  if (p.h_a) {
    const int h4 = p.H >> 2;
    for (int64_t e = tid; e < R * h4; e += nthr) {
      const int n = (int)((e / h4) / p.M);
      const float keep = env_done(p, n) ? 0.f : 1.f;
      float4 a = reinterpret_cast<const float4 *>(p.h_a)[e], c = reinterpret_cast<const float4 *>(p.h_c)[e];
      a.x *= keep; a.y *= keep; a.z *= keep; a.w *= keep;
      c.x *= keep; c.y *= keep; c.z *= keep; c.w *= keep;
      reinterpret_cast<float4 *>(p.ha_dst)[e] = a;
      reinterpret_cast<float4 *>(p.hc_dst)[e] = c;
    }
  }
}
```

### mappo_amd/csrc/mlp.hip

```cpp
#include "mlp_host.h"
#include "mlp_upd.h"
#include "mlp_upd2.h"
#include "mlp_upd16.h"
#include <stdlib.h>

#ifdef MLP_STAMPS
static unsigned long long *g_stamp_host = nullptr;
static unsigned long long *g_stamp_waves_host = nullptr;
extern "C" int mappo_debug_set_stamps(unsigned long long *buf) { g_stamp_host = buf; return 0; }
extern "C" int mappo_debug_set_stamps_waves(unsigned long long *buf) { g_stamp_waves_host = buf; return 0; }
#endif

extern "C" int64_t mappo_net_param_count(const mappo_net_desc *desc) {
  if (!desc) return -1;
  return net_offsets(*desc).total;
}

template <int MODE>
static int launch_forward(const FwdArgs &a_in, hipStream_t st, const char *who) {
  MAPPO_CLEAR_STICKY();
  const int64_t n_tiles = (a_in.B + TS - 1) / TS;
  const int LN = a_in.desc.layer_N;
  const int nw = fit_waves(a_in.desc, n_tiles >= 4 ? 4 : (n_tiles >= 2 ? 2 : 1));
  FwdArgs a = a_in;
  a.off = net_offsets(a.desc);
  a.map = lds_map(a.desc, nw);
  const size_t lds_bytes = (size_t)a.map.total * sizeof(float);
  MAPPO_REQUIRE(lds_bytes <= LDS_DYN_MAX, "%s: needs %zu B of LDS", who, lds_bytes);
  int64_t nb = (n_tiles + nw - 1) / nw;
  if (nb > NUM_CU) nb = NUM_CU;
  dim3 grid((unsigned)nb), block(WAVE * nw);
  {
    if (a.desc.in_dim > MAXD && a.desc.in_dim <= 512 && a.x_M == 0) {
      Wide16Args w;
      size_t lb;
      dim3 g2, b2;
      if (int rcp = wide_forward_prepare(a, w, lb, g2, b2, who)) return rcp;
      const int64_t nt16 = (a.B + 15) / 16;
      int64_t sk_max = WIDE_SK_MAX_TILES;
      if (const char *e = getenv("MAPPO_WIDE_SK_TILES")) sk_max = atoll(e);
      if (nt16 <= sk_max && !getenv("MAPPO_WIDE_NO_SK")) {
        const int64_t gsk = nt16 < NUM_CU ? nt16 : NUM_CU;
        if (int rcw = wide16_launch_forward_sk(MODE, a.desc.use_relu != 0, LN, dim3((unsigned)gsk), lb, st, w, a, who)) return rcw;
        MAPPO_CHECK_LAUNCH(who);
        return MAPPO_OK;
      }
      FwdArgs ar = a;
      ar.map = lds_map_tail(a.desc);
      const size_t lres = sizeof(float) * ((size_t)HID * 64 * ((a.desc.in_dim + 63) / 64) + HID + ar.map.tiles);
      if (MODE == 2 && LN <= 1 && nt16 >= 2 * 8 * NUM_CU && lres <= 159 * 1024 &&
          !(getenv("MAPPO_WIDE_RESIDENT") && atoi(getenv("MAPPO_WIDE_RESIDENT")) == 0)) {
        const int rcr = a.desc.use_relu ? wide16_launch_features_resident_r<true>(LN, g2, st, w, ar) : wide16_launch_features_resident_r<false>(LN, g2, st, w, ar);
        if (rcr) return rcr;
        MAPPO_CHECK_LAUNCH(who);
        return MAPPO_OK;
      }
      if (int rcw = wide16_launch_forward(MODE, a.desc.use_relu != 0, LN, g2, b2, lb, st, w, a, who)) return rcw;
      MAPPO_CHECK_LAUNCH(who);
      return MAPPO_OK;
    }
  }
  const int xw = a.desc.in_dim > MAXD ? 2 : (a.desc.in_dim > 32 ? 1 : 0);
  constexpr int prof_id = (MODE == 1) ? MAPPO_PROF_ACT : MAPPO_PROF_MLP_FWD;
  if (int rc = dispatch_relu_ln(a.desc.use_relu != 0, LN, [&](auto R, auto L) {
        if (xw == 2) return launch_kernel<mlp_forward_kernel<R.value, L.value, MODE, 2>, LDS_DYN_MAX, prof_id>(who, grid, block, lds_bytes, st, a);
        if (xw == 1) return launch_kernel<mlp_forward_kernel<R.value, L.value, MODE, 1>, LDS_DYN_MAX, prof_id>(who, grid, block, lds_bytes, st, a);
        return launch_kernel<mlp_forward_kernel<R.value, L.value, MODE, 0>, LDS_DYN_MAX, prof_id>(who, grid, block, lds_bytes, st, a);
      }))
    return rc;
  MAPPO_CHECK_LAUNCH(who);
  return MAPPO_OK;
}

extern "C" int mappo_mlp_forward(const float *params, const mappo_net_desc *desc, const float *x, const int32_t *rows,
                                 int64_t B, float *out, mappo_stream_t stream) {
  if (int rc = check_desc(desc, "mlp_forward")) return rc;
  MAPPO_REQUIRE(params && x && out && B > 0, "mlp_forward: bad arguments");
  FwdArgs a = {};
  a.params = params; a.x = x; a.rows = rows; a.out = out; a.desc = *desc; a.B = B;
  return launch_forward<0>(a, as_stream(stream), "mlp_forward");
}

extern "C" int mappo_mlp_features(const float *params, const mappo_net_desc *desc, const float *x, const int32_t *rows,
                                  int64_t B, float *featT, mappo_stream_t stream) {
  if (int rc = check_desc_trunk(desc, "mlp_features")) return rc;
  MAPPO_REQUIRE(params && x && featT && B > 0, "mlp_features: bad arguments");
  FwdArgs a = {};
  a.params = params; a.x = x; a.rows = rows; a.out = featT; a.desc = *desc; a.B = B;
  if (desc->in_dim <= MAXD) return launch_features16(a, as_stream(stream));
  return launch_forward<2>(a, as_stream(stream), "mlp_features");
}

int mlp_features_blocked_wide_(const float *params, const mappo_net_desc *desc, const float *x, const int32_t *rows, int64_t B,
                               float *out_blocked, mappo_stream_t stream) {
  if (int rc = check_desc_trunk(desc, "mlp_features_seq")) return rc;
  MAPPO_REQUIRE(desc->in_dim > MAXD && desc->in_dim <= 512 && (B & 15) == 0, "mlp_features_seq: wide inputs need in_dim <= 512 and Nc %% 16 == 0");
  FwdArgs a = {};
  a.params = params; a.x = x; a.rows = rows; a.out = out_blocked; a.desc = *desc; a.B = B; a.out_blocked = 1;
  return launch_forward<2>(a, as_stream(stream), "mlp_features_seq");
}

extern "C" int mappo_actor_act(const float *params, const mappo_net_desc *desc, const float *obs, const float *avail,
                               int64_t B, int32_t deterministic, uint64_t seed, uint64_t counter,
                               const uint64_t *counter_dev, float *actions, float *logp, mappo_stream_t stream) {
  if (int rc = check_desc(desc, "actor_act")) return rc;
  MAPPO_REQUIRE(params && obs && actions && logp && B > 0, "actor_act: bad arguments");
  FwdArgs a = {};
  a.params = params; a.x = obs; a.rows = nullptr; a.avail = avail; a.actions = actions; a.logp = logp; a.desc = *desc;
  a.B = B; a.deterministic = deterministic; a.seed = seed; a.counter = counter; a.counter_dev = counter_dev;
  return launch_forward<1>(a, as_stream(stream), "actor_act");
}

extern "C" int mappo_actor_act_md(const float *params, const mappo_net_desc *desc, const float *obs, const float *avail,
                                  const int32_t *head_dims, int32_t n_heads, int64_t B, int32_t deterministic, uint64_t seed,
                                  uint64_t counter, const uint64_t *counter_dev, float *actions, float *logp, mappo_stream_t stream) {
  MdHeads md;
  if (int rc = check_md(desc, head_dims, n_heads, avail, "actor_act_md", md)) return rc;
  MAPPO_REQUIRE(params && obs && actions && logp && B > 0, "actor_act_md: bad arguments");
  MAPPO_CLEAR_STICKY();
  FwdArgs a = {};
  a.params = params; a.x = obs; a.actions = actions; a.logp = logp; a.desc = *desc;
  a.B = B; a.deterministic = deterministic; a.seed = seed; a.counter = counter; a.counter_dev = counter_dev;
  const int64_t n_tiles = (B + TS - 1) / TS;
  const int nw = fit_waves(a.desc, n_tiles >= 4 ? 4 : (n_tiles >= 2 ? 2 : 1));
  a.off = net_offsets(a.desc);
  a.map = lds_map(a.desc, nw);
  const size_t lds_bytes = (size_t)a.map.total * sizeof(float);
  MAPPO_REQUIRE(lds_bytes <= LDS_DYN_MAX, "actor_act_md: needs %zu B of LDS", lds_bytes);
  int64_t nb = (n_tiles + nw - 1) / nw;
  if (nb > NUM_CU) nb = NUM_CU;
  dim3 grid((unsigned)nb), block(WAVE * nw);
  const bool xw = a.desc.in_dim > 32;
  hipStream_t st = as_stream(stream);
  if (int rc = dispatch_relu_ln<1>(a.desc.use_relu != 0, a.desc.layer_N, [&](auto R, auto L) {
        if (xw) return launch_kernel<mlp_forward_md_kernel<R.value, L.value, 1>, LDS_DYN_MAX, MAPPO_PROF_ACT>("actor_act_md", grid, block, lds_bytes, st, a, md);
        return launch_kernel<mlp_forward_md_kernel<R.value, L.value, 0>, LDS_DYN_MAX, MAPPO_PROF_ACT>("actor_act_md", grid, block, lds_bytes, st, a, md);
      }))
    return rc;
  MAPPO_CHECK_LAUNCH("actor_act_md");
  return MAPPO_OK;
}

#define UPD16_WAVES (UPD16_THREADS / WAVE)
static size_t upd16_lds_floats(const mappo_net_desc &d, bool actor) {
  const bool w = d.in_dim > 32;
  if (actor) {
    if (d.layer_N > 0) return w ? L16<1, 1, true>::TOTAL : L16<1, 1, false>::TOTAL;
    return w ? L16<0, 1, true>::TOTAL : L16<0, 1, false>::TOTAL;
  }
  if (d.layer_N > 0) return w ? L16<1, 2, true>::TOTAL : L16<1, 2, false>::TOTAL;
  return w ? L16<0, 2, true>::TOTAL : L16<0, 2, false>::TOTAL;
}
static bool upd16_eligible(const mappo_net_desc &d, bool actor) {
  return d.in_dim <= MAXD && d.layer_N <= 1 && !d.recurrent && (actor ? d.out_dim <= 16 : d.out_dim == 1) &&
         upd16_lds_floats(d, actor) * sizeof(float) <= UPD16_LDS_MAX;
}
// ... 432 lines not shown
#pragma unroll
    for (int j = 0; j < 2; ++j)
#pragma unroll
      for (int r = 0; r < 16; ++r) gW[i][j][r] = 0.f;
  }
  const int64_t n_tiles = (p.B + TS - 1) / TS;
  for (int64_t tile = (int64_t)blockIdx.x * 4 + wave; tile < n_tiles; tile += (int64_t)gridDim.x * 4) {
    const int64_t base = tile * TS;
    const int n_valid = (int)min((int64_t)TS, p.B - base);
    const bool ok = l31 < n_valid;
    {
      float v[HID / 2];
      const int64_t col = base + min(l31, n_valid - 1);
#pragma unroll
      for (int i = 0; i < HID / 2; ++i) v[i] = dz1T[(int64_t)(2 * i + half) * p.B + col];
#pragma unroll
      for (int i = 0; i < HID / 2; ++i) tD[(2 * i + half) * TP + l31] = ok ? v[i] : 0.f;
    }
    const int64_t row = ok ? (p.rows ? (int64_t)p.rows[base + l31] : base + l31) : 0;
    const float mean0 = ok ? stats[base + l31] : 0.f, rstd0 = ok ? stats[p.B + base + l31] : 1.f;
    wide_commit_chunk(tXc, p.x + row * D, D, c0, ok, mean0, rstd0, l31, half);
    wave_lds_sync();
    {
      const float g0 = sG[l31], b0 = sBt[l31], g1 = sG[32 + l31], b1 = sBt[32 + l31];
#pragma unroll 2
      for (int ss = 0; ss < TS / 2; ++ss) {
        const int s = 2 * ss + half;
        const float a0 = tD[l31 * TP + s], a1 = tD[(32 + l31) * TP + s];
        const float x0 = tXc[l31 * TP + s] * g0 + b0, x1 = tXc[(32 + l31) * TP + s] * g1 + b1;
        gW[0][0] = mfma(a0, x0, gW[0][0]);
        gW[0][1] = mfma(a0, x1, gW[0][1]);
        gW[1][0] = mfma(a1, x0, gW[1][0]);
        gW[1][1] = mfma(a1, x1, gW[1][1]);
      }
    }
    if (p.use_feature_norm) {
      f32x16 dX[2];
#pragma unroll
      for (int t = 0; t < 2; ++t)
#pragma unroll
        for (int r = 0; r < 16; ++r) dX[t][r] = 0.f;
#pragma unroll 4
      for (int ff = 0; ff < HID / 2; ++ff) {
        const int f = 2 * ff + half;
        const float b = tD[f * TP + l31];
        dX[0] = mfma(sW[l31 * WP + f], b, dX[0]);
        dX[1] = mfma(sW[(32 + l31) * WP + f], b, dX[1]);
      }
#pragma unroll
      for (int t = 0; t < 2; ++t)
#pragma unroll
        for (int r = 0; r < 16; ++r) {
          accB[t][r] += dX[t][r];
          accG[t][r] += dX[t][r] * tXc[(32 * t + ROWMAP(r, half)) * TP + l31];
        }
    }
    wave_lds_sync();
  }
  float gFnB = 0.f, gFnW = 0.f;
  if (p.use_feature_norm) {
    wave_lds_sync();
#pragma unroll
    for (int t = 0; t < 2; ++t)
#pragma unroll
      for (int r = 0; r < 16; ++r) {
        tD[(32 * t + ROWMAP(r, half)) * TP + l31] = accB[t][r];
        tXc[(32 * t + ROWMAP(r, half)) * TP + l31] = accG[t][r];
      }
    wave_lds_sync();
    for (int j = 0; j < TS; ++j) { gFnB += tD[lane * TP + j]; gFnW += tXc[lane * TP + j]; }
  }
  __syncthreads();
  float *red = sBt + MAXD;
  for (int w = 0; w < 4; ++w) {
    if (wave == w) {
#pragma unroll
      for (int ti = 0; ti < 2; ++ti)
#pragma unroll
        for (int tj = 0; tj < 2; ++tj) {
          float old[16];
#pragma unroll
          for (int r = 0; r < 16; ++r) old[r] = (w == 0) ? 0.f : red[(32 * ti + ROWMAP(r, half)) * MAXD + 32 * tj + l31];
#pragma unroll
          for (int r = 0; r < 16; ++r) red[(32 * ti + ROWMAP(r, half)) * MAXD + 32 * tj + l31] = old[r] + gW[ti][tj][r];
        }
      const float ob = (w == 0) ? 0.f : red[HID * MAXD + lane], og = (w == 0) ? 0.f : red[HID * MAXD + MAXD + lane];
      red[HID * MAXD + lane] = ob + gFnB;
      red[HID * MAXD + MAXD + lane] = og + gFnW;
    }
    __syncthreads();
  }
  float *slab = p.slabs + (size_t)blockIdx.x * p.slab_stride + p.slab_col0;
  for (int e = threadIdx.x; e < HID * kc; e += blockDim.x) {
    const int f = e / kc, kk = e - f * kc;
    slab[p.off.w1 + f * D + c0 + kk] = red[f * MAXD + kk];
  }
  if (p.use_feature_norm)
    for (int e = threadIdx.x; e < kc; e += blockDim.x) {
      slab[p.off.fn_b + c0 + e] = red[HID * MAXD + e];
      slab[p.off.fn_w + c0 + e] = red[HID * MAXD + MAXD + e];
    }
}

extern "C" int64_t mappo_wide_workspace_floats(int64_t B) { return wide_z1_offset(B) + (int64_t)HID * B; }

extern "C" int32_t mappo_wide_l1_slabs(int64_t B) {
  return mappo_mlp_backward_slabs(B);
}

extern "C" int mappo_wide_l1_backward(const float *params, const mappo_net_desc *desc, const float *x, const int32_t *rows,
                                      int64_t B, const float *wide_ws, float *slabs, int64_t slab_stride, int64_t slab_col0,
                                      int32_t layout, mappo_stream_t stream) {
  if (int rc = check_desc_trunk(desc, "wide_l1_backward")) return rc;
  MAPPO_REQUIRE(desc->in_dim > MAXD, "wide_l1_backward: in_dim %d is handled inside the update kernels", desc->in_dim);
  MAPPO_REQUIRE(params && x && wide_ws && slabs && B > 0, "wide_l1_backward: bad arguments");
  MAPPO_REQUIRE(layout == MAPPO_WIDE_LAYOUT_BLOCKED || layout == MAPPO_WIDE_LAYOUT_FEATURE_MAJOR,
                "wide_l1_backward: layout %d (pass mappo_wide_layout(desc, producer) of the launch that filled the workspace)", (int)layout);
  MAPPO_REQUIRE(layout != MAPPO_WIDE_LAYOUT_BLOCKED || desc->in_dim <= 512, "wide_l1_backward: the blocked layout exists for in_dim <= 512 only");
  {
    if (layout == MAPPO_WIDE_LAYOUT_BLOCKED) {
      const NetOff o = net_offsets(*desc);
      MAPPO_REQUIRE(slab_col0 >= 0 && slab_col0 + o.total <= slab_stride, "wide_l1_backward: slab column range");
      WideBwd16Args w = {};
      w.params = params; w.x = x; w.rows = rows; w.wide_ws = wide_ws; w.slabs = slabs; w.slab_stride = slab_stride; w.slab_col0 = slab_col0;
      w.B = B; w.D = desc->in_dim; w.w1 = o.w1; w.fn_w = desc->use_feature_norm ? o.fn_w : -1; w.fn_b = desc->use_feature_norm ? o.fn_b : -1;
      const int nch = (desc->in_dim + 63) / 64;
      w.nca = nch <= 2 ? 2 : (nch <= 4 ? 4 : 8);
      const int rows_max = mappo_mlp_backward_slabs(B);
      w.groups = 8 / w.nca;
      if (rows_max < w.groups) w.groups = 1;
      const int gx = rows_max / w.groups;
      (void)wide16_launch_l1_bwd(w, dim3((unsigned)gx), as_stream(stream));
      MAPPO_CHECK_LAUNCH("wide_l1_backward");
      return MAPPO_OK;
    }
  }
  MAPPO_CLEAR_STICKY();
  WideArgs a = {};
  a.params = params; a.x = x; a.rows = rows; a.wide_ws = wide_ws; a.slabs = slabs; a.slab_stride = slab_stride; a.slab_col0 = slab_col0;
  a.off = net_offsets(*desc); a.B = B; a.D = desc->in_dim; a.use_feature_norm = desc->use_feature_norm;
  MAPPO_REQUIRE(slab_col0 >= 0 && slab_col0 + a.off.total <= slab_stride, "wide_l1_backward: slab column range");
  const size_t lds_bytes = (size_t)(MAXD * WP + 2 * MAXD + 4 * 2 * HID * TP) * sizeof(float);
  dim3 grid((unsigned)mappo_wide_l1_slabs(B), (unsigned)((desc->in_dim + MAXD - 1) / MAXD));
  if (int rc = launch_kernel<wide_l1_bwd_kernel, LDS_DYN_MAX>("wide_l1_backward", grid, dim3(256), lds_bytes, as_stream(stream), a)) return rc;
  MAPPO_CHECK_LAUNCH("wide_l1_backward");
  return MAPPO_OK;
}

__global__ __launch_bounds__(256) void update_stats_kernel(const double *__restrict__ pa, const double *__restrict__ pc, int na,
                                                          int nc, const double *__restrict__ mb_moments, int use_policy_active,
                                                          int use_value_active, double *__restrict__ stats,
                                                          double *__restrict__ acc) {
  __shared__ double smem[16 * 4];
  double v[4] = {0.0, 0.0, 0.0, 0.0};
  for (int b = threadIdx.x; b < na; b += blockDim.x) { v[0] += pa[b * 4 + 0]; v[1] += pa[b * 4 + 1]; v[2] += pa[b * 4 + 2]; }
  for (int b = threadIdx.x; b < nc; b += blockDim.x) v[3] += pc[b * 4 + 0];
  block_sum<4>(v, smem);
  if (threadIdx.x == 0) {
    const double sa = mb_moments[2] > 0.0 ? mb_moments[2] : 1.0;
    const double Bg = mb_moments[3] > 0.0 ? mb_moments[3] : 1.0;
    const double den_pi = use_policy_active ? sa : Bg, den_v = use_value_active ? sa : Bg;
    stats[0] = v[3] / den_v;
    stats[1] = -v[0] / den_pi;
    stats[2] = v[1] / den_pi;
    stats[3] = v[2] / Bg;
    stats[4] = mb_moments[2];
    stats[5] = mb_moments[3];
    if (acc) { acc[0] += stats[0]; acc[1] += stats[1]; acc[2] += stats[2]; acc[3] += stats[3]; }
  }
}

extern "C" int mappo_update_stats(const double *actor_partials, int32_t n_actor, const double *critic_partials,
                                  int32_t n_critic, const double *mb_moments, const mappo_ppo_cfg *cfg, double *stats,
                                  double *acc, mappo_stream_t stream) {
  MAPPO_REQUIRE(critic_partials && mb_moments && cfg && stats && n_critic > 0 && n_actor >= 0, "update_stats: bad arguments");
  hipLaunchKernelGGL(update_stats_kernel, dim3(1), dim3(256), 0, as_stream(stream), actor_partials, critic_partials,
                     actor_partials ? (int)n_actor : 0, (int)n_critic, mb_moments, cfg->use_policy_active_masks,
                     cfg->use_value_active_masks, stats, acc);
  MAPPO_CHECK_LAUNCH("update_stats");
  return MAPPO_OK;
}

__global__ void selftest_mfma_kernel(const float *A, const float *Bm, float *Dm) {
  const int lane = threadIdx.x, l31 = lane & 31, half = lane >> 5;
  f32x16 acc;
#pragma unroll
  for (int r = 0; r < 16; ++r) acc[r] = 0.f;
  acc = mfma(A[l31 * 2 + half], Bm[half * 32 + l31], acc);
#pragma unroll
  for (int r = 0; r < 16; ++r) Dm[ROWMAP(r, half) * 32 + l31] = acc[r];
}

extern "C" int mappo_selftest_mfma(const float *A, const float *Bm, float *D, mappo_stream_t stream) {
  MAPPO_REQUIRE(A && Bm && D, "selftest_mfma: null pointer");
  hipLaunchKernelGGL(selftest_mfma_kernel, dim3(1), dim3(WAVE), 0, as_stream(stream), A, Bm, D);
  MAPPO_CHECK_LAUNCH("selftest_mfma");
  return MAPPO_OK;
}
```

### mappo_amd/csrc/stats.hip

```cpp
#include "common.h"

#define STAT_BLOCK 256
#define STAT_MAX_BLOCKS 1024

static inline int stat_blocks(int64_t n) {
  int64_t b = (n + STAT_BLOCK * 4 - 1) / (STAT_BLOCK * 4);
  if (b < 1) b = 1;
  if (b > STAT_MAX_BLOCKS) b = STAT_MAX_BLOCKS;
  return (int)b;
}

template <int NV>
__global__ __launch_bounds__(STAT_BLOCK) void final_reduce_kernel(const double *__restrict__ partials, int nblk,
                                                                 double *__restrict__ out, double extra) {
  __shared__ double smem[16 * NV];
  double v[NV];
#pragma unroll
  for (int i = 0; i < NV; ++i) v[i] = 0.0;
  for (int b = threadIdx.x; b < nblk; b += blockDim.x) {
#pragma unroll
    for (int i = 0; i < NV; ++i) v[i] += partials[(size_t)b * NV + i];
  }
  block_sum<NV>(v, smem);
  if (threadIdx.x == 0) {
#pragma unroll
    for (int i = 0; i < NV; ++i) out[i] = v[i];
    if (extra >= 0.0) out[NV] = extra;
  }
}

__global__ __launch_bounds__(STAT_BLOCK) void adv_moments_kernel(const float *__restrict__ returns,
                                                                const float *__restrict__ value_preds,
                                                                const float *__restrict__ active,
                                                                const float *__restrict__ vn_state,
                                                                float *__restrict__ adv, double *__restrict__ partials,
                                                                int64_t n) {
  __shared__ double smem[16 * 3];
  const VnStats vn = vn_stats(vn_state);
  double v[3] = {0.0, 0.0, 0.0};
  const int64_t stride = (int64_t)gridDim.x * blockDim.x;
  for (int64_t i = (int64_t)blockIdx.x * blockDim.x + threadIdx.x; i < n; i += stride) {
    const float a = returns[i] - (value_preds[i] * vn.sd + vn.mean);
    adv[i] = a;
    if (active[i] != 0.f) {
      v[0] += (double)a;
      v[1] += (double)a * (double)a;
      v[2] += 1.0;
    }
  }
  block_sum<3>(v, smem);
  if (threadIdx.x == 0) {
    partials[blockIdx.x * 3 + 0] = v[0];
    partials[blockIdx.x * 3 + 1] = v[1];
    partials[blockIdx.x * 3 + 2] = v[2];
  }
}

__global__ __launch_bounds__(STAT_BLOCK) void adv_normalize_kernel(float *__restrict__ adv,
                                                                  const double *__restrict__ moments, int64_t n) {
  const double cnt = moments[2] > 0.0 ? moments[2] : 1.0;
  const double mean_d = moments[0] / cnt;
  double var_d = moments[1] / cnt - mean_d * mean_d;
  if (var_d < 0.0) var_d = 0.0;
  const float mean = (float)mean_d;
  const float denom = (float)sqrt(var_d) + 1e-5f;
  const int64_t stride = (int64_t)gridDim.x * blockDim.x;
  for (int64_t i = (int64_t)blockIdx.x * blockDim.x + threadIdx.x; i < n; i += stride)
    adv[i] = (adv[i] - mean) / denom;
}

extern "C" int64_t mappo_adv_workspace_bytes(int64_t n) { return (int64_t)STAT_MAX_BLOCKS * 3 * sizeof(double); }

extern "C" int mappo_adv_moments(const float *returns, const float *value_preds, const float *active_masks,
                                 const float *vn_state, float *adv, double *moments, void *workspace, int64_t n,
                                 mappo_stream_t stream) {
  MAPPO_REQUIRE(n > 0 && returns && value_preds && active_masks && adv && moments && workspace,
                "adv_moments: bad arguments (n=%lld)", (long long)n);
  const int nblk = stat_blocks(n);
  hipLaunchKernelGGL(adv_moments_kernel, dim3(nblk), dim3(STAT_BLOCK), 0, as_stream(stream), returns, value_preds,
                     active_masks, vn_state, adv, (double *)workspace, n);
  hipLaunchKernelGGL(final_reduce_kernel<3>, dim3(1), dim3(STAT_BLOCK), 0, as_stream(stream),
                     (const double *)workspace, nblk, moments, -1.0);
  MAPPO_CHECK_LAUNCH("adv_moments");
  return MAPPO_OK;
}

extern "C" int mappo_adv_normalize(float *adv, const double *moments, int64_t n, mappo_stream_t stream) {
  MAPPO_REQUIRE(n > 0 && adv && moments, "adv_normalize: bad arguments");
  hipLaunchKernelGGL(adv_normalize_kernel, dim3(stat_blocks(n)), dim3(STAT_BLOCK), 0, as_stream(stream), adv,
                     moments, n);
  MAPPO_CHECK_LAUNCH("adv_normalize");
  return MAPPO_OK;
}

__global__ __launch_bounds__(STAT_BLOCK) void minibatch_moments_kernel(const float *__restrict__ returns,
                                                                      const float *__restrict__ active,
                                                                      const int32_t *__restrict__ rows, int64_t B,
                                                                      double *__restrict__ partials) {
  __shared__ double smem[16 * 3];
  double v[3] = {0.0, 0.0, 0.0};
  const int64_t stride = (int64_t)gridDim.x * blockDim.x;
  for (int64_t i = (int64_t)blockIdx.x * blockDim.x + threadIdx.x; i < B; i += stride) {
    const int64_t row = rows ? (int64_t)rows[i] : i;
    const float r = returns[row];
    v[0] += (double)r;
    v[1] += (double)r * (double)r;
    v[2] += (double)active[row];
  }
  block_sum<3>(v, smem);
  if (threadIdx.x == 0) {
    partials[blockIdx.x * 3 + 0] = v[0];
    partials[blockIdx.x * 3 + 1] = v[1];
    partials[blockIdx.x * 3 + 2] = v[2];
  }
}

extern "C" int64_t mappo_moments_workspace_bytes(int64_t B) { return (int64_t)STAT_MAX_BLOCKS * 3 * sizeof(double); }

extern "C" int mappo_minibatch_moments(const float *returns, const float *active_masks, const int32_t *rows, int64_t B,
                                       double *mb_moments, void *workspace, mappo_stream_t stream) {
  MAPPO_REQUIRE(B > 0 && returns && active_masks && mb_moments && workspace, "minibatch_moments: bad arguments");
  const int nblk = stat_blocks(B);
  hipLaunchKernelGGL(minibatch_moments_kernel, dim3(nblk), dim3(STAT_BLOCK), 0, as_stream(stream), returns,
                     active_masks, rows, B, (double *)workspace);
  hipLaunchKernelGGL(final_reduce_kernel<3>, dim3(1), dim3(STAT_BLOCK), 0, as_stream(stream),
                     (const double *)workspace, nblk, mb_moments, (double)B);
  MAPPO_CHECK_LAUNCH("minibatch_moments");
  return MAPPO_OK;
}

__global__ void valuenorm_update_kernel(float *vn_state, const double *mb_moments, float w, float omw) {
  const double B = mb_moments[3] > 0.0 ? mb_moments[3] : 1.0;
  const float bm = (float)(mb_moments[0] / B);
  const float bsq = (float)(mb_moments[1] / B);
  vn_state[0] = __fadd_rn(__fmul_rn(vn_state[0], w), __fmul_rn(bm, omw));
  vn_state[1] = __fadd_rn(__fmul_rn(vn_state[1], w), __fmul_rn(bsq, omw));
  vn_state[2] = __fadd_rn(__fmul_rn(vn_state[2], w), omw);
}

extern "C" int mappo_valuenorm_update(float *vn_state, const double *mb_moments, double beta, mappo_stream_t stream) {
  MAPPO_REQUIRE(vn_state && mb_moments, "valuenorm_update: null pointer");
  hipLaunchKernelGGL(valuenorm_update_kernel, dim3(1), dim3(1), 0, as_stream(stream), vn_state, mb_moments,
                     (float)beta, (float)(1.0 - beta));
  MAPPO_CHECK_LAUNCH("valuenorm_update");
  return MAPPO_OK;
}

__global__ void valuenorm_update_n_kernel(float *vn_state, const double *mb_moments, float w, float omw, int n, float *states_out) {
  const double B = mb_moments[3] > 0.0 ? mb_moments[3] : 1.0;
  const float bm = (float)(mb_moments[0] / B);
  const float bsq = (float)(mb_moments[1] / B);
  float s0 = vn_state[0], s1 = vn_state[1], s2 = vn_state[2];
  for (int e = 0; e < n; ++e) {
    s0 = __fadd_rn(__fmul_rn(s0, w), __fmul_rn(bm, omw));
    s1 = __fadd_rn(__fmul_rn(s1, w), __fmul_rn(bsq, omw));
    s2 = __fadd_rn(__fmul_rn(s2, w), omw);
    states_out[3 * e + 0] = s0; states_out[3 * e + 1] = s1; states_out[3 * e + 2] = s2;
  }
  vn_state[0] = s0; vn_state[1] = s1; vn_state[2] = s2;
}

extern "C" int mappo_valuenorm_update_n(float *vn_state, const double *mb_moments, double beta, int32_t n, float *states_out,
                                        mappo_stream_t stream) {
  MAPPO_REQUIRE(vn_state && mb_moments && states_out && n >= 1, "valuenorm_update_n: bad arguments");
  hipLaunchKernelGGL(valuenorm_update_n_kernel, dim3(1), dim3(1), 0, as_stream(stream), vn_state, mb_moments, (float)beta,
                     (float)(1.0 - beta), (int)n, states_out);
  MAPPO_CHECK_LAUNCH("valuenorm_update_n");
  return MAPPO_OK;
}
```

### mappo_amd/ops.py

```python
import ctypes as C

import torch

from . import _lib
from ._lib import NetDesc, PpoCfg


def _ptr(t, dtype=torch.float32, allow_none=False):
    if t is None:
        if allow_none:
            return None
        raise ValueError("tensor required")
    if not t.is_cuda:
        raise _lib.MappoHipError("mappo_amd ops need tensors in HBM (cuda/hip device); got a CPU tensor — "
                                 "there is no CPU fallback")
    if t.dtype != dtype:
        raise TypeError(f"expected {dtype}, got {t.dtype}")
    if not t.is_contiguous():
        raise ValueError("tensor must be contiguous")
    return C.c_void_p(t.data_ptr())


def _stream():
    return C.c_void_p(torch.cuda.current_stream().cuda_stream)
# ... 311 lines not shown
    f64 = torch.float64
    arr, K = _heads(head_dims)
    rc = _lib.load().mappo_rollout_episode_reference(_ptr(actor_params), C.byref(actor_desc), _ptr(critic_params), C.byref(critic_desc), arr, K,
                                                     int(T), int(N), int(env_episode_length), int(env_seed) & (2 ** 64 - 1),
                                                     _ptr(agent_pos, f64), _ptr(agent_vel, f64), _ptr(landmark_pos, f64),
                                                     _ptr(goal, torch.int32), _ptr(tstep, torch.int32), _ptr(episode, torch.int64),
                                                     int(bool(deterministic)), int(seed) & (2 ** 64 - 1), int(counter) & (2 ** 64 - 1),
                                                     _ptr(counter_dev, torch.int64, allow_none=True), _ptr(obs_buf), _ptr(share_buf),
                                                     _ptr(rew_buf), _ptr(mask_buf), _ptr(actions), _ptr(logp), _ptr(values), _ptr(next_values),
                                                     int(bool(centralized)), _stream())
    _lib.check(rc, "mappo_rollout_episode_reference")


def comm_agent(actor_params, actor_desc, critic_params, critic_desc, seed, counter_dev, obs_buf, share_buf, rew_buf, mask_buf, actions, logp, values,
               next_values):
    ag = _lib.CommAgent()
    ag.actor_params, ag.critic_params = _ptr(actor_params).value, _ptr(critic_params).value
    ag.actor_desc, ag.critic_desc = actor_desc, critic_desc
    ag.seed = int(seed) & (2 ** 64 - 1)
    cd = _ptr(counter_dev, torch.int64, allow_none=True)
    ag.counter_dev = cd.value if cd is not None else None
    for name, t in (("obs_buf", obs_buf), ("share_buf", share_buf), ("rew_buf", rew_buf), ("mask_buf", mask_buf), ("actions", actions),
                    ("logp", logp), ("values", values), ("next_values", next_values)):
        setattr(ag, name, _ptr(t).value)
    return ag


def rollout_episode_comm(speaker, listener, T, N, env_episode_length, env_seed, listener_pos, listener_vel, landmark_pos, goal, symbol,
                         tstep, episode, deterministic, counter, centralized):
    f64 = torch.float64
    rc = _lib.load().mappo_rollout_episode_comm(C.byref(speaker), C.byref(listener), int(T), int(N), int(env_episode_length),
                                                int(env_seed) & (2 ** 64 - 1), _ptr(listener_pos, f64), _ptr(listener_vel, f64),
                                                _ptr(landmark_pos, f64), _ptr(goal, torch.int32), _ptr(symbol, torch.int32),
                                                _ptr(tstep, torch.int32), _ptr(episode, torch.int64), int(bool(deterministic)),
                                                int(counter) & (2 ** 64 - 1), int(bool(centralized)), _stream())
    _lib.check(rc, "mappo_rollout_episode_comm")


def rollout_episode_adversary(agents, T, N, env_episode_length, env_seed, agent_pos, agent_vel, landmark_pos, goal, tstep, episode,
                              deterministic, counter, centralized):
    if len(agents) != 3:
        raise ValueError(f"rollout_episode_adversary: simple_adversary is built for num_agents = 3 (got {len(agents)} agents)")
    f64 = torch.float64
    arr = (_lib.CommAgent * 3)(*agents)
    rc = _lib.load().mappo_rollout_episode_adversary(arr, _ptr(agent_pos, f64), _ptr(agent_vel, f64), _ptr(landmark_pos, f64),
                                                     _ptr(goal, torch.int32), _ptr(tstep, torch.int32), _ptr(episode, torch.int64), int(T),
                                                     int(N), int(env_episode_length), int(env_seed) & (2 ** 64 - 1),
                                                     int(bool(deterministic)), int(counter) & (2 ** 64 - 1), int(bool(centralized)),
                                                     _stream())
    _lib.check(rc, "mappo_rollout_episode_adversary")


def mlp_backward_slabs(B):
    return int(_lib.load().mappo_mlp_backward_slabs(int(B)))


PRODUCER_MLP_BACKWARD, PRODUCER_ACTOR_UPDATE, PRODUCER_CRITIC_UPDATE, PRODUCER_TRUNK_BACKWARD = 0, 1, 2, 3


def wide_layout(desc, producer):
    v = int(_lib.load().mappo_wide_layout(C.byref(desc), int(producer)))
    if v < 0:
        _lib.check(v, "mappo_wide_layout")
    return v


def _wide(desc, x, rows, B, slabs, slab_stride, slab_col0, params, wide_ws, producer):
    if wide_ws is not None:
        rc = _lib.load().mappo_wide_l1_backward(_ptr(params), C.byref(desc), _ptr(x), _ptr(rows, torch.int32, allow_none=True), int(B),
                                                _ptr(wide_ws), _ptr(slabs), int(slab_stride), int(slab_col0),
                                                wide_layout(desc, producer), _stream())
        _lib.check(rc, "mappo_wide_l1_backward")


_wide_ws_cache = {}


def wide_workspace(desc, B, device):
    if desc.in_dim <= 64:
        return None
    key = (int(B), str(device), int(torch.cuda.current_stream().cuda_stream))
    ws = _wide_ws_cache.get(key)
    if ws is None:
        ws = torch.empty(int(_lib.load().mappo_wide_workspace_floats(int(B))), dtype=torch.float32, device=device)
        _wide_ws_cache[key] = ws
    return ws


def wide_l1_slabs(B):
    return int(_lib.load().mappo_wide_l1_slabs(int(B)))


def mlp_backward(params, desc, x, rows, B, dout, slabs, slab_stride, slab_col0):
    ws = wide_workspace(desc, B, x.device)
    rc = _lib.load().mappo_mlp_backward(_ptr(params), C.byref(desc), _ptr(x), _ptr(rows, torch.int32, allow_none=True),
                                        int(B), _ptr(dout), _ptr(slabs), int(slab_stride), int(slab_col0),
                                        _ptr(ws, allow_none=True), _stream())
    _lib.check(rc, "mappo_mlp_backward")
    _wide(desc, x, rows, B, slabs, slab_stride, slab_col0, params, ws, PRODUCER_MLP_BACKWARD)


def update_partials(device):
    return torch.zeros(int(_lib.load().mappo_update_partials_bytes()) // 8, dtype=torch.float64, device=device)


def actor_update(params, desc, obs, rows, B, avail, actions, old_logp, adv, active, mb_moments, cfg, slabs, slab_stride,
                 slab_col0, partials, n_blocks=0):
    ws = wide_workspace(desc, B, obs.device)
    rc = _lib.load().mappo_actor_update(_ptr(params), C.byref(desc), _ptr(obs), _ptr(rows, torch.int32, allow_none=True), int(B),
                                        _ptr(avail, allow_none=True), _ptr(actions), _ptr(old_logp), _ptr(adv), _ptr(active),
                                        _ptr(mb_moments, torch.float64), C.byref(cfg), _ptr(slabs), int(slab_stride),
                                        int(slab_col0), _ptr(partials, torch.float64), _ptr(ws, allow_none=True), int(n_blocks),
                                        _stream())
    _lib.check(rc, "mappo_actor_update")
    _wide(desc, obs, rows, B, slabs, slab_stride, slab_col0, params, ws, PRODUCER_ACTOR_UPDATE)


def critic_update(params, desc, share_obs, rows, B, v_old, returns, active, vn_state, mb_moments, cfg, slabs, slab_stride,
                  slab_col0, partials, n_blocks=0):
    ws = wide_workspace(desc, B, share_obs.device)
    rc = _lib.load().mappo_critic_update(_ptr(params), C.byref(desc), _ptr(share_obs), _ptr(rows, torch.int32, allow_none=True),
                                         int(B), _ptr(v_old), _ptr(returns), _ptr(active), _ptr(vn_state, allow_none=True),
                                         _ptr(mb_moments, torch.float64), C.byref(cfg), _ptr(slabs), int(slab_stride),
                                         int(slab_col0), _ptr(partials, torch.float64), _ptr(ws, allow_none=True), int(n_blocks),
                                         _stream())
    _lib.check(rc, "mappo_critic_update")
    _wide(desc, share_obs, rows, B, slabs, slab_stride, slab_col0, params, ws, PRODUCER_CRITIC_UPDATE)


def dual_update_slabs(actor_desc, critic_desc, B):
    return int(_lib.load().mappo_dual_update_slabs(C.byref(actor_desc), C.byref(critic_desc), int(B)))


def actor_critic_update(actor_params, actor_desc, obs, critic_params, critic_desc, share_obs, rows, B, avail, actions, old_logp, adv,
                        active, v_old, returns, vn_state, mb_moments, cfg, slabs, slab_stride, actor_col0, critic_col0,
                        actor_partials, critic_partials):
    rc = _lib.load().mappo_actor_critic_update(_ptr(actor_params), C.byref(actor_desc), _ptr(obs), _ptr(critic_params), C.byref(critic_desc),
                                               _ptr(share_obs), _ptr(rows, torch.int32, allow_none=True), int(B),
                                               _ptr(avail, allow_none=True), _ptr(actions), _ptr(old_logp), _ptr(adv), _ptr(active),
                                               _ptr(v_old), _ptr(returns), _ptr(vn_state, allow_none=True),
                                               _ptr(mb_moments, torch.float64), C.byref(cfg), _ptr(slabs), int(slab_stride),
                                               int(actor_col0), int(critic_col0), _ptr(actor_partials, torch.float64),
                                               _ptr(critic_partials, torch.float64), _stream())
    _lib.check(rc, "mappo_actor_critic_update")


def update_stats(actor_partials, n_actor, critic_partials, n_critic, mb_moments, cfg, stats, acc=None):
    rc = _lib.load().mappo_update_stats(_ptr(actor_partials, torch.float64, allow_none=True), int(n_actor),
                                        _ptr(critic_partials, torch.float64), int(n_critic), _ptr(mb_moments, torch.float64),
                                        C.byref(cfg), _ptr(stats, torch.float64), _ptr(acc, torch.float64, allow_none=True), _stream())
    _lib.check(rc, "mappo_update_stats")


def mlp_features(params, desc, x, rows, B, featT):
    rc = _lib.load().mappo_mlp_features(_ptr(params), C.byref(desc), _ptr(x), _ptr(rows, torch.int32, allow_none=True), int(B),
                                        _ptr(featT), _stream())
    _lib.check(rc, "mappo_mlp_features")


def gru_forward(params, desc, featT, h0, h0_rows, masks, rows, L, Nc, h_last=None, head_mode=0, out=None,
                avail=None, deterministic=False, seed=0, counter=0, counter_dev=None, actions=None, logp=None):
    rc = _lib.load().mappo_gru_forward(_ptr(params), C.byref(desc), _ptr(featT), _ptr(h0),
                                       _ptr(h0_rows, torch.int32, allow_none=True),
                                       _ptr(masks), _ptr(rows, torch.int32, allow_none=True), int(L), int(Nc),
                                       _ptr(h_last, allow_none=True), int(head_mode),
                                       _ptr(out, allow_none=True), _ptr(avail, allow_none=True), int(bool(deterministic)),
                                       int(seed) & (2 ** 64 - 1), int(counter) & (2 ** 64 - 1),
                                       _ptr(counter_dev, torch.int64, allow_none=True), _ptr(actions, allow_none=True),
                                       _ptr(logp, allow_none=True), _stream())
    _lib.check(rc, "mappo_gru_forward")


def gru_step_dual(actor_params, actor_desc, actor_featT, actor_h0, actor_h_last, critic_params, critic_desc, critic_featT, critic_h0,
                  critic_h_last, masks, Nc, avail, deterministic, seed, counter, counter_dev, actions, logp, values):
    rc = _lib.load().mappo_gru_step_dual(_ptr(actor_params), C.byref(actor_desc), _ptr(actor_featT), _ptr(actor_h0), _ptr(actor_h_last),
                                         _ptr(critic_params), C.byref(critic_desc), _ptr(critic_featT), _ptr(critic_h0),
                                         _ptr(critic_h_last), _ptr(masks), int(Nc), _ptr(avail, allow_none=True), int(bool(deterministic)),
                                         int(seed) & (2 ** 64 - 1), int(counter) & (2 ** 64 - 1),
                                         _ptr(counter_dev, torch.int64, allow_none=True), _ptr(actions), _ptr(logp), _ptr(values), _stream())
    _lib.check(rc, "mappo_gru_step_dual")


def recurrent_step_dual(actor_params, actor_desc, actor_obs, actor_h0, actor_h_last, critic_params, critic_desc, critic_obs, critic_h0,
                  critic_h_last, masks, Nc, avail, deterministic, seed, counter, counter_dev, actions, logp, values):
    rc = _lib.load().mappo_recurrent_step_dual(_ptr(actor_params), C.byref(actor_desc), _ptr(actor_obs), _ptr(actor_h0), _ptr(actor_h_last),
                                         _ptr(critic_params), C.byref(critic_desc), _ptr(critic_obs), _ptr(critic_h0),
                                         _ptr(critic_h_last), _ptr(masks), int(Nc), _ptr(avail, allow_none=True), int(bool(deterministic)),
                                         int(seed) & (2 ** 64 - 1), int(counter) & (2 ** 64 - 1),
                                         _ptr(counter_dev, torch.int64, allow_none=True), _ptr(actions), _ptr(logp), _ptr(values), _stream())
    _lib.check(rc, "mappo_recurrent_step_dual")


def mlp_features_dual(params_a, desc_a, x_a, featT_a, params_c, desc_c, x_c, featT_c, B):
    rc = _lib.load().mappo_mlp_features_dual(_ptr(params_a), C.byref(desc_a), _ptr(x_a), _ptr(featT_a), _ptr(params_c), C.byref(desc_c),
                                             _ptr(x_c), _ptr(featT_c), int(B), _stream())
    _lib.check(rc, "mappo_mlp_features_dual")


def trunk_backward(params, desc, x, rows, B, dxT, slabs, slab_stride, slab_col0):
    ws = wide_workspace(desc, B, x.device)
    rc = _lib.load().mappo_trunk_backward(_ptr(params), C.byref(desc), _ptr(x), _ptr(rows, torch.int32, allow_none=True), int(B),
                                          _ptr(dxT), _ptr(slabs), int(slab_stride), int(slab_col0), _ptr(ws, allow_none=True), _stream())
    _lib.check(rc, "mappo_trunk_backward")
    _wide(desc, x, rows, B, slabs, slab_stride, slab_col0, params, ws, PRODUCER_TRUNK_BACKWARD)


def gru16_scratch_floats(L, Nc):
    return int(_lib.load().mappo_gru16_scratch_floats(int(L), int(Nc)))


def gru16_blocked_floats(L, Nc):
    return int(_lib.load().mappo_gru16_blocked_floats(int(L), int(Nc)))


def gru16_slabs(L, Nc):
    return int(_lib.load().mappo_gru16_slabs(int(L), int(Nc)))


def mlp_features_seq(params, desc, x, rows, L, Nc, out_blocked):
    rc = _lib.load().mappo_mlp_features_seq(_ptr(params), C.byref(desc), _ptr(x), _ptr(rows, torch.int32, allow_none=True), int(L), int(Nc),
                                            _ptr(out_blocked), _stream())
    _lib.check(rc, "mappo_mlp_features_seq")


def gru16_forward_loss(params, desc, x, x_blocked, h0, h0_rows, masks, rows, L, Nc, head, avail, actions, old_logp, adv, active, v_old,
                       returns, vn_state, mb_moments, cfg, scratch, slabs, slab_stride, slab_col0, partials):
    o = lambda t: _ptr(t, allow_none=True)
    rc = _lib.load().mappo_gru16_forward_loss(_ptr(params), C.byref(desc), _ptr(x), int(bool(x_blocked)), _ptr(h0),
                                              _ptr(h0_rows, torch.int32, allow_none=True), _ptr(masks),
                                              _ptr(rows, torch.int32, allow_none=True), int(L), int(Nc), int(head), o(avail), o(actions),
                                              o(old_logp), o(adv), _ptr(active), o(v_old), o(returns), o(vn_state),
                                              _ptr(mb_moments, torch.float64), C.byref(cfg), _ptr(scratch), _ptr(slabs), int(slab_stride),
                                              int(slab_col0), _ptr(partials, torch.float64), _stream())
    _lib.check(rc, "mappo_gru16_forward_loss")


def gru16_backward(params, desc, masks, rows, L, Nc, scratch, dxT=None):
    rc = _lib.load().mappo_gru16_backward(_ptr(params), C.byref(desc), _ptr(masks), _ptr(rows, torch.int32, allow_none=True), int(L), int(Nc),
                                          _ptr(scratch), _ptr(dxT, allow_none=True), _stream())
    _lib.check(rc, "mappo_gru16_backward")


def gru16_wgrad(desc, x, x_blocked, scratch, L, Nc, slabs, slab_stride, slab_col0):
    rc = _lib.load().mappo_gru16_wgrad(C.byref(desc), _ptr(x), int(bool(x_blocked)), _ptr(scratch), int(L), int(Nc), _ptr(slabs),
                                       int(slab_stride), int(slab_col0), _stream())
    _lib.check(rc, "mappo_gru16_wgrad")


def trunk_backward_seq(params, desc, x, rows, L, Nc, dx_blocked, slabs, slab_stride, slab_col0):
    ws = wide_workspace(desc, L * Nc, x.device)
    rc = _lib.load().mappo_trunk_backward_seq(_ptr(params), C.byref(desc), _ptr(x), _ptr(rows, torch.int32, allow_none=True), int(L), int(Nc),
                                              _ptr(dx_blocked), _ptr(slabs), int(slab_stride), int(slab_col0), _ptr(ws, allow_none=True),
                                              _stream())
    _lib.check(rc, "mappo_trunk_backward_seq")
    _wide(desc, x, rows, L * Nc, slabs, slab_stride, slab_col0, params, ws, PRODUCER_TRUNK_BACKWARD)


def slab_reduce(slabs, n_slabs, slab_stride, P, grad):
    rc = _lib.load().mappo_slab_reduce(_ptr(slabs), int(n_slabs), int(slab_stride), int(P), _ptr(grad), _stream())
    _lib.check(rc, "mappo_slab_reduce")


def optim_workspace(P, device):
    return _ws(_lib.load().mappo_optim_workspace_bytes(int(P)), device)


def clip_adam(params, grad, exp_avg, exp_avg_sq, seg_bounds, opt_hyper, opt_step, grad_norms, workspace, norm_acc=None):
    n_seg = len(seg_bounds) - 1
    arr = (C.c_int64 * (n_seg + 1))(*[int(b) for b in seg_bounds])
    rc = _lib.load().mappo_clip_adam(_ptr(params), _ptr(grad), _ptr(exp_avg), _ptr(exp_avg_sq), arr, n_seg,
                                     _ptr(opt_hyper), _ptr(opt_step, torch.int32), _ptr(grad_norms),
                                     _ptr(norm_acc, torch.float64, allow_none=True), _ptr(workspace, torch.uint8), _stream())
    _lib.check(rc, "mappo_clip_adam")


def reduce_clip_adam(slabs, n_slabs, slab_stride, params, grad, exp_avg, exp_avg_sq, seg_bounds, opt_hyper, opt_step, grad_norms,
                     workspace, norm_acc=None):
    n_seg = len(seg_bounds) - 1
    arr = (C.c_int64 * (n_seg + 1))(*[int(b) for b in seg_bounds])
    rc = _lib.load().mappo_reduce_clip_adam(_ptr(slabs), int(n_slabs), int(slab_stride), _ptr(params), _ptr(grad), _ptr(exp_avg),
                                            _ptr(exp_avg_sq), arr, n_seg, _ptr(opt_hyper), _ptr(opt_step, torch.int32), _ptr(grad_norms),
                                            _ptr(norm_acc, torch.float64, allow_none=True), _ptr(workspace, torch.uint8), _stream())
    _lib.check(rc, "mappo_reduce_clip_adam")


def selftest_mfma(A, Bm, D):
    rc = _lib.load().mappo_selftest_mfma(_ptr(A), _ptr(Bm), _ptr(D), _stream())
    _lib.check(rc, "mappo_selftest_mfma")


PROF_IDS = dict(gae=0, ppo_loss=1, mlp_fwd=2, mlp_bwd=3, slab_reduce=4, adam=5, act=6)


def profile_arm(kernel, start_event, stop_event):
    for ev in (start_event, stop_event):
        if ev.cuda_event == 0:
            ev.record()
    rc = _lib.load().mappo_profile_arm(PROF_IDS[kernel], C.c_void_p(start_event.cuda_event), C.c_void_p(stop_event.cuda_event))
    _lib.check(rc, "mappo_profile_arm")


def mpe_spread_reset(agent_pos, agent_vel, landmark_pos, tstep, episode, obs, N, M, L, seed):
    f64 = torch.float64
    rc = _lib.load().mappo_mpe_spread_reset(_ptr(agent_pos, f64), _ptr(agent_vel, f64), _ptr(landmark_pos, f64), _ptr(tstep, torch.int32),
                                            _ptr(episode, torch.int64), _ptr(obs),
                                            int(N), int(M), int(L), int(seed) & (2 ** 64 - 1), _stream())
# ... 85 lines not shown
```

### mappo_amd/utils/shared_buffer.py

```python
import numpy as np
import torch

from .. import ops
from .util import obs_dim_of, get_shape_from_act_space, to_device_f32


class SharedReplayBuffer(object):
    def __init__(self, args, num_agents, obs_space, cent_obs_space, act_space, device=None):
        self.episode_length = args.episode_length
        self.n_rollout_threads = args.n_rollout_threads
        self.num_agents = num_agents
        self.hidden_size = args.hidden_size
        self.recurrent_N = args.recurrent_N
        self.gamma = args.gamma
        self.gae_lambda = args.gae_lambda
        self._use_gae = args.use_gae
        self._use_popart = args.use_popart
        self._use_valuenorm = args.use_valuenorm
        self._use_proper_time_limits = args.use_proper_time_limits
        self.device = torch.device(device if device is not None else "cuda")
        self.perm_device = getattr(args, "perm_device", "cuda")

        T, N, M, H = self.episode_length, self.n_rollout_threads, num_agents, self.hidden_size
        obs_dim, share_dim = obs_dim_of(obs_space), obs_dim_of(cent_obs_space)
        z = lambda *s: torch.zeros(s, dtype=torch.float32, device=self.device)
        o = lambda *s: torch.ones(s, dtype=torch.float32, device=self.device)
        self.share_obs = z(T + 1, N, M, share_dim)
        self.obs = z(T + 1, N, M, obs_dim)
        self.rnn_states = z(T + 1, N, M, self.recurrent_N, H)
        self.rnn_states_critic = z(T + 1, N, M, self.recurrent_N, H)
        self.value_preds = z(T + 1, N, M, 1)
        self.returns = z(T + 1, N, M, 1)
        if act_space.__class__.__name__ == "Discrete":
            self.available_actions = o(T + 1, N, M, act_space.n)
        else:
            self.available_actions = None
        act_shape = get_shape_from_act_space(act_space)
        self.actions = z(T, N, M, act_shape)
        self.action_log_probs = z(T, N, M, act_shape)
        self.rewards = z(T, N, M, 1)
        self.masks = o(T + 1, N, M, 1)
        self.bad_masks = o(T + 1, N, M, 1)
        self.active_masks = o(T + 1, N, M, 1)
        self.device = self.obs.device
        self.step = 0

    def _put(self, dst, src):
        if torch.is_tensor(src) and src.device == dst.device:
            if src.shape != dst.shape:
                src = src.reshape(dst.shape) if src.numel() == dst.numel() else src.expand(dst.shape)
            dst.copy_(src)
        else:
            dst.copy_(to_device_f32(src, self.device).view(dst.shape), non_blocking=True)

    def insert(self, share_obs, obs, rnn_states_actor, rnn_states_critic, actions, action_log_probs, value_preds, rewards,
               masks, bad_masks=None, active_masks=None, available_actions=None):
        s = self.step
        self._put(self.share_obs[s + 1], share_obs)
        self._put(self.obs[s + 1], obs)
        self._put(self.rnn_states[s + 1], rnn_states_actor)
        self._put(self.rnn_states_critic[s + 1], rnn_states_critic)
        self._put(self.actions[s], actions)
        self._put(self.action_log_probs[s], action_log_probs)
        self._put(self.value_preds[s], value_preds)
        self._put(self.rewards[s], rewards)
        self._put(self.masks[s + 1], masks)
        if bad_masks is not None:
            self._put(self.bad_masks[s + 1], bad_masks)
        if active_masks is not None:
            self._put(self.active_masks[s + 1], active_masks)
        if available_actions is not None:
            self._put(self.available_actions[s + 1], available_actions)
        self.step = (s + 1) % self.episode_length

    def insert_env(self, share_obs, obs, rewards, masks, rnn_states_actor=None, rnn_states_critic=None, bad_masks=None,
                   active_masks=None, available_actions=None):
        s = self.step
        self._put(self.share_obs[s + 1], share_obs)
        self._put(self.obs[s + 1], obs)
        self._put(self.rewards[s], rewards)
        self._put(self.masks[s + 1], masks)
        if rnn_states_actor is not None:
            self._put(self.rnn_states[s + 1], rnn_states_actor)
        if rnn_states_critic is not None:
            self._put(self.rnn_states_critic[s + 1], rnn_states_critic)
        if bad_masks is not None:
            self._put(self.bad_masks[s + 1], bad_masks)
        if active_masks is not None:
            self._put(self.active_masks[s + 1], active_masks)
        if available_actions is not None:
            self._put(self.available_actions[s + 1], available_actions)
        self.step = (s + 1) % self.episode_length

    def insert_smac_fused(self, share_obs, obs, rewards, dones, bad_transition, available_actions, rnn_states=None,
                          rnn_states_critic=None):
        dev = self.device
        f32 = lambda t, d: (torch.is_tensor(t) and t.device == dev and t.dtype == torch.float32 and t.is_contiguous() and t.dim() == 3
                            and t.shape[-1] == d)
        ok = (f32(obs, self.obs.shape[-1]) and f32(share_obs, self.share_obs.shape[-1]) and torch.is_tensor(rewards)
              and rewards.device == dev and rewards.dtype == torch.float32 and rewards.dim() in (2, 3)
              and torch.is_tensor(dones) and dones.device == dev and dones.dtype == torch.bool and dones.dim() == 2
              and (bad_transition is None or (torch.is_tensor(bad_transition) and bad_transition.device == dev
                                              and bad_transition.dtype == torch.bool and bad_transition.is_contiguous()
                                              and bad_transition.numel() == dones.numel()))
              and (available_actions is None or (self.available_actions is not None
                                                 and f32(available_actions, self.available_actions.shape[-1]))))
        if rnn_states is not None:
            state_ok = lambda h: (torch.is_tensor(h) and h.device == dev and h.dtype == torch.float32 and h.is_contiguous()
                                  and h.numel() == self.rnn_states[0].numel() and h.data_ptr() % 16 == 0)
            ok = ok and state_ok(rnn_states) and state_ok(rnn_states_critic) and (self.recurrent_N * self.rnn_states.shape[-1]) % 4 == 0
        if not ok:
            return False
        s = self.step
        ops.insert_smac(obs, share_obs, available_actions, rewards, dones, bad_transition, rnn_states, rnn_states_critic, self.obs[s + 1],
                        self.share_obs[s + 1], self.available_actions[s + 1] if available_actions is not None else None,
                        self.rewards[s], self.masks[s + 1], self.bad_masks[s + 1], self.active_masks[s + 1],
                        self.rnn_states[s + 1] if rnn_states is not None else None,
                        self.rnn_states_critic[s + 1] if rnn_states is not None else None)
        self.step = (s + 1) % self.episode_length
        return True

    def insert_mpe_fused(self, obs, rewards, dones, centralized, rnn_states=None, rnn_states_critic=None):
        ok = (torch.is_tensor(obs) and torch.is_tensor(rewards) and torch.is_tensor(dones) and obs.device == self.device
              and obs.dtype == torch.float32 and obs.dim() == 3 and obs.stride(2) == 1 and rewards.device == self.device
              and rewards.dtype == torch.float32 and dones.device == self.device and dones.dtype == torch.bool and dones.dim() == 2)
        if rnn_states is not None:
            state_ok = lambda h: (torch.is_tensor(h) and h.device == self.device and h.dtype == torch.float32 and h.is_contiguous()
                                  and h.numel() == self.rnn_states[0].numel() and h.data_ptr() % 16 == 0)
            ok = ok and state_ok(rnn_states) and state_ok(rnn_states_critic) and (self.recurrent_N * self.rnn_states.shape[-1]) % 4 == 0
        if not ok:
            return False
        s = self.step
        if rnn_states is not None:
            ops.insert_mpe_rnn(obs, rewards, dones, self.obs[s + 1], self.share_obs[s + 1], self.rewards[s], self.masks[s + 1],
                               centralized, rnn_states, rnn_states_critic, self.rnn_states[s + 1], self.rnn_states_critic[s + 1])
        else:
            ops.insert_mpe(obs, rewards, dones, self.obs[s + 1], self.share_obs[s + 1], self.rewards[s], self.masks[s + 1], centralized)
        self.step = (s + 1) % self.episode_length
        return True

    def chooseinsert(self, share_obs, obs, rnn_states, rnn_states_critic, actions, action_log_probs, value_preds, rewards,
                     masks, bad_masks=None, active_masks=None, available_actions=None):
        s = self.step
        self._put(self.share_obs[s], share_obs)
        self._put(self.obs[s], obs)
        self._put(self.rnn_states[s + 1], rnn_states)
        self._put(self.rnn_states_critic[s + 1], rnn_states_critic)
        self._put(self.actions[s], actions)
        self._put(self.action_log_probs[s], action_log_probs)
        self._put(self.value_preds[s], value_preds)
        self._put(self.rewards[s], rewards)
        self._put(self.masks[s + 1], masks)
        if bad_masks is not None:
            self._put(self.bad_masks[s + 1], bad_masks)
        if active_masks is not None:
            self._put(self.active_masks[s], active_masks)
        if available_actions is not None:
            self._put(self.available_actions[s], available_actions)
        self.step = (s + 1) % self.episode_length

    def after_update(self):
        arrs = [a for a in (self.share_obs, self.obs, self.rnn_states, self.rnn_states_critic, self.masks, self.bad_masks,
                            self.active_masks, self.available_actions) if a is not None]
        ops.copy_batch([(a[0], a[-1]) for a in arrs])

    def chooseafter_update(self):
        for arr in (self.rnn_states, self.rnn_states_critic, self.masks, self.bad_masks):
            arr[0].copy_(arr[-1])

    def compute_returns(self, next_value, value_normalizer=None):
        T = self.episode_length
        R = self.n_rollout_threads * self.num_agents
        nv = to_device_f32(next_value, self.device).reshape(R)
        vn_state = None
        if self._use_popart:
            raise NotImplementedError("use_popart: PopArt.update raises in the reference itself (SURVEY.md §8c)")
        if self._use_valuenorm:
            if value_normalizer is None:
                raise ValueError("use_valuenorm needs the trainer's value_normalizer")
            vn_state = value_normalizer.state
        ops.gae_scan(self.rewards.view(T, R), self.value_preds.view(T + 1, R), nv, self.masks.view(T + 1, R),
                     self.bad_masks.view(T + 1, R), self.returns.view(T + 1, R), vn_state, self.gamma, self.gae_lambda,
                     self._use_gae, self._use_proper_time_limits)

    def _randperm(self, n):
        if self.perm_device == "cpu":
            return torch.randperm(n).to(self.device, non_blocking=True)
        return torch.randperm(n, device=self.device)

    def _dims(self):
        T, N, M = self.episode_length, self.n_rollout_threads, self.num_agents
        return T, N * M

    def feed_forward_rows(self, num_mini_batch=None, mini_batch_size=None, rand=None):
        T, R = self._dims()
        batch_size = T * R
        if mini_batch_size is None:
            assert batch_size >= num_mini_batch, (
                f"PPO requires the number of processes ({self.n_rollout_threads}) * number of steps ({T}) * number of "
                f"agents ({self.num_agents}) = {batch_size} to be greater than or equal to the number of PPO mini "
                f"batches ({num_mini_batch}).")
            mini_batch_size = batch_size // num_mini_batch
        if rand is None:
            rand = self._randperm(batch_size)
        rand = torch.as_tensor(rand, device=self.device)
        return [rand[i * mini_batch_size:(i + 1) * mini_batch_size].to(torch.int32).contiguous()
                for i in range(num_mini_batch)]

    def recurrent_rows(self, num_mini_batch, data_chunk_length, rand=None):
        T, R = self._dims()
        L = data_chunk_length
        data_chunks = (T * R) // L
        mbs = data_chunks // num_mini_batch
        if rand is None:
            rand = self._randperm(data_chunks)
        rand = torch.as_tensor(rand, device=self.device).to(torch.int64)
        steps = torch.arange(L, device=self.device, dtype=torch.int64)
        out = []
        for k in range(num_mini_batch):
            c = rand[k * mbs:(k + 1) * mbs]
            q = (c[None, :] * L + steps[:, None]).reshape(-1)
            rows = (q % T) * R + q // T
            q0 = c * L
            h0 = (q0 % T) * R + q0 // T
            out.append((rows.to(torch.int32).contiguous(), h0.to(torch.int32).contiguous()))
        return out

    def recurrent_rows_epochs(self, n_epochs, num_mini_batch, data_chunk_length):
        T, R = self._dims()
        data_chunks = (T * R) // data_chunk_length
        e_idx = torch.arange(n_epochs, device=self.device, dtype=torch.float64)[:, None]
        keys = torch.rand(n_epochs, data_chunks, device=self.device, dtype=torch.float64) + e_idx
        perm = keys.view(-1).argsort().view(n_epochs, data_chunks) - (e_idx * data_chunks).to(torch.int64)
        rows, h0 = ops.recurrent_rows(perm, data_chunk_length, T, R, num_mini_batch)
        return [[(rows[e, k], h0[e, k]) for k in range(num_mini_batch)] for e in range(n_epochs)]

    def naive_recurrent_rows(self, num_mini_batch, perm=None):
        T, R = self._dims()
        assert R >= num_mini_batch, (
            f"PPO requires the number of processes ({self.n_rollout_threads})* number of agents ({self.num_agents}) "
            f"to be greater than or equal to the number of PPO mini batches ({num_mini_batch}).")
        n = R // num_mini_batch
        if perm is None:
            perm = self._randperm(R)
        perm = torch.as_tensor(perm, device=self.device).to(torch.int64)
        t = torch.arange(T, device=self.device, dtype=torch.int64)
        out = []
        for start in range(0, R, n):
            cols = perm[start:start + n]
            if cols.numel() < n:
                break
            rows = (t[:, None] * R + cols[None, :]).reshape(-1)
            out.append((rows.to(torch.int32).contiguous(), cols.to(torch.int32).contiguous()))
        return out

    def _flat(self, arr):
        T = self.episode_length
        return arr[:T].reshape(T * self.n_rollout_threads * self.num_agents, *arr.shape[3:])

    def _sample(self, rows, advantages, h0_rows=None):
        rows = rows.long()
        hr = rows if h0_rows is None else h0_rows.long()
        g = lambda a: self._flat(a)[rows]
        adv = torch.as_tensor(advantages, device=self.device, dtype=torch.float32).reshape(-1, 1)
        avail = g(self.available_actions) if self.available_actions is not None else None
        return (g(self.share_obs), g(self.obs), self._flat(self.rnn_states)[hr], self._flat(self.rnn_states_critic)[hr],
                g(self.actions), g(self.value_preds), g(self.returns), g(self.masks), g(self.active_masks),
                g(self.action_log_probs), adv[rows], avail)

    def feed_forward_generator(self, advantages, num_mini_batch=None, mini_batch_size=None):
        for rows in self.feed_forward_rows(num_mini_batch, mini_batch_size):
            yield self._sample(rows, advantages)

    def recurrent_generator(self, advantages, num_mini_batch, data_chunk_length):
        for rows, h0 in self.recurrent_rows(num_mini_batch, data_chunk_length):
            yield self._sample(rows, advantages, h0)

    def naive_recurrent_generator(self, advantages, num_mini_batch):
        for rows, cols in self.naive_recurrent_rows(num_mini_batch):
            yield self._sample(rows, advantages, cols)
```

Before: 79.06 million agent-steps/s.

## Fuse once-per-train glue into a prologue and an epilogue kernel

The advantage computation, the advantage and minibatch moment reductions (a last-block ticket does the final reduce), the ValueNorm multi-epoch update and the zeroing of the statistics buffer now run in a single prologue launch. A single epilogue launch computes the update statistics and performs the after_update buffer copies, with block 0 doing the stats and the other blocks doing the copies. This removes several small launches and host-side calls per train() on the single-process whole-buffer path. It adds a grid-wide atomic ticket pattern with fences, which needs correct memory ordering, and a new opt-out flag.

```diff
diff --git a/include/mappo_hip.h b/include/mappo_hip.h
--- a/include/mappo_hip.h
+++ b/include/mappo_hip.h
@@ -195,6 +195,15 @@
                        double *acc ,
                        mappo_stream_t stream);
 
+int64_t mappo_train_prologue_workspace_bytes(int64_t n);
+int mappo_train_prologue(const float *returns , const float *value_preds , const float *active_masks ,
+                         float *vn_state , float *adv , double *adv_moments ,
+                         double *mb_moments , double beta, int32_t n_epochs, float *states_out ,
+                         double *zero, int64_t n_zero, void *workspace, int32_t *ticket, int64_t n, mappo_stream_t stream);
+int mappo_train_epilogue(const double *actor_partials, int32_t n_actor, const double *critic_partials, int32_t n_critic,
+                         const double *mb_moments, const mappo_ppo_cfg *cfg , double *stats , double *acc,
+                         int32_t count, float *const *dst, const float *const *src, const int64_t *n_floats, mappo_stream_t stream);
+
 int mappo_mlp_features(const float *params, const mappo_net_desc *desc , const float *x, const int32_t *rows,
                        int64_t B, float *featT , mappo_stream_t stream);
 int mappo_gru_forward(const float *params, const mappo_net_desc *desc , const float *featT, const float *h0,
diff --git a/mappo_amd/_lib.py b/mappo_amd/_lib.py
--- a/mappo_amd/_lib.py
+++ b/mappo_amd/_lib.py
@@ -86,6 +86,10 @@
     "mappo_actor_critic_update_md": (C.c_int, [_P, C.POINTER(NetDesc), _P, _P, C.POINTER(NetDesc), _P, _P, _I64, _P, C.POINTER(_I32), _I32,
                                                _P, _P, _P, _P, _P, _P, _P, _P, C.POINTER(PpoCfg), _P, _I64, _I64, _I64, _P, _P, _P]),
     "mappo_update_stats": (C.c_int, [_P, _I32, _P, _I32, _P, C.POINTER(PpoCfg), _P, _P, _P]),
+    "mappo_train_prologue_workspace_bytes": (_I64, [_I64]),
+    "mappo_train_prologue": (C.c_int, [_P, _P, _P, _P, _P, _P, _P, _D, _I32, _P, _P, _I64, _P, _P, _I64, _P]),
+    "mappo_train_epilogue": (C.c_int, [_P, _I32, _P, _I32, _P, C.POINTER(PpoCfg), _P, _P, _I32, C.POINTER(C.c_void_p),
+                                       C.POINTER(C.c_void_p), C.POINTER(_I64), _P]),
     "mappo_mlp_features": (C.c_int, [_P, C.POINTER(NetDesc), _P, _P, _I64, _P, _P]),
     "mappo_gru_forward": (C.c_int, [_P, C.POINTER(NetDesc), _P, _P, _P, _P, _P, _I32, _I32, _P, _I32, _P, _P, _I32, _U64, _U64,
                                     _P, _P, _P, _P]),
diff --git a/mappo_amd/algorithms/r_mappo/r_mappo.py b/mappo_amd/algorithms/r_mappo/r_mappo.py
--- a/mappo_amd/algorithms/r_mappo/r_mappo.py
+++ b/mappo_amd/algorithms/r_mappo/r_mappo.py
@@ -36,6 +36,7 @@
         self._fused = not bool(getattr(args, "unfused_update", False))
         self._use_graph = bool(getattr(args, "use_hip_graph", True))
         self._concurrent_update = bool(getattr(args, "concurrent_update", False))
+        self._fuse_glue = bool(getattr(args, "fuse_train_glue", True))
         self._graphs = {}
         self._dp_graphs = {}
         self._graph_buffers = {}
@@ -273,9 +274,6 @@
     def _train_body(self, buffer, update_actor, after_update):
         T = buffer.episode_length
         S = T * buffer.n_rollout_threads * buffer.num_agents
-        adv = self.compute_advantages(buffer)
-        src, _ = self._buffer_sources(buffer, adv)
-        self._zbuf.zero_()
         whole = self.num_mini_batch == 1 and not self._exact_order
         dp_graph = self._dist is not None and self._use_graph and whole and self._fused and self._dist.world_is_gpu
         key = (self._buffer_key(buffer), bool(update_actor))
@@ -283,6 +281,13 @@
         if whole and self._fused and (self._dist is None or dp_graph) and not self._concurrent_update \
                 and os.environ.get("MAPPO_EPOCH_BATCH", "1") != "0":
             self._epochs = dict(n=self.ppo_epoch, e=0, states=self._buf("vn_states", (self.ppo_epoch, 3)))
+        glue = self._fuse_glue and self._epochs is not None and self._dist is None
+        if glue:
+            adv = self._train_prologue(buffer)
+        else:
+            adv = self.compute_advantages(buffer)
+            self._zbuf.zero_()
+        src, _ = self._buffer_sources(buffer, adv)
         if dp_graph:
             vn_state = self.value_normalizer.state if self._use_valuenorm else None
             self._moments(src, None, S, vn_state)
@@ -319,12 +324,18 @@
                         st.replay()
                     self._update(src, rows, B, update_actor, moments_ready=True, part="optim")
                 else:
-                    self._update(src, rows, B, update_actor, moments_ready=whole and epoch > 0)
+                    self._update(src, rows, B, update_actor, moments_ready=glue or (whole and epoch > 0))
         if self._epochs is not None:
             n_rows = ops.dual_update_slabs(self.policy.actor.desc, self.policy.critic.desc, S) if (update_actor and self._dual_update and self.policy.can_dual_update()) \
                 else ops.mlp_backward_slabs(S)
-            ops.update_stats(self._pa if update_actor else None, n_rows, self._pc, n_rows, self._mb_moments, self._cfg, self._stats,
-                             self._acc)
+            pairs = buffer.after_update_pairs() if (glue and after_update) else None
+            if pairs:
+                ops.train_epilogue(self._pa if update_actor else None, n_rows, self._pc, n_rows, self._mb_moments, self._cfg,
+                                   self._stats, self._acc, pairs)
+                after_update = False
+            else:
+                ops.update_stats(self._pa if update_actor else None, n_rows, self._pc, n_rows, self._mb_moments, self._cfg,
+                                 self._stats, self._acc)
             self._epochs = None
         if dp_graph and self._dp_graphs.get(key) is None:
             self._dp_graphs[key] = "warm"
@@ -344,11 +355,27 @@
         ops.adv_normalize(adv, self._adv_moments)
         return adv
 
+    def _train_prologue(self, buffer):
+        T = buffer.episode_length
+        S = T * buffer.n_rollout_threads * buffer.num_agents
+        adv = self._buf("adv", (S,))
+        if self._glue_ws is None:
+            self._glue_ws = ops.train_prologue_workspace(S, self.device)
+        vn = self.value_normalizer if self._use_valuenorm else None
+        ep = self._epochs
+        ops.train_prologue(buffer.returns[:T].view(S), buffer.value_preds[:T].view(S), buffer.active_masks[:T].view(S),
+                           vn.state if vn is not None else None, adv, self._adv_moments, self._mb_moments,
+                           vn.beta if vn is not None else 0.0, ep["n"], ep["states"] if vn is not None else None, self._zbuf, *self._glue_ws)
+        ops.adv_normalize(adv, self._adv_moments)
+        return adv
+
+    _glue_ws = None
+
     def _finish_train_info(self):
         num_updates = self.ppo_epoch * self.num_mini_batch
         if self._dist is not None:
             self._dist.all_reduce_sum_(self._acc[:4])
-        acc = (self._acc / max(num_updates, 1)).cpu().numpy()
+        acc = self._acc.cpu().numpy() * (np.float64(1.0) / np.float64(max(num_updates, 1)))
         return dict(value_loss=float(acc[0]), policy_loss=float(acc[1]), dist_entropy=float(acc[2]),
                     actor_grad_norm=float(acc[4]), critic_grad_norm=float(acc[5]), ratio=float(acc[3]))
 
diff --git a/mappo_amd/config.py b/mappo_amd/config.py
--- a/mappo_amd/config.py
+++ b/mappo_amd/config.py
@@ -91,6 +91,11 @@
                         "steps run inside that launch too (mappo_rollout_episode_spread), and so they do with the GPU-resident simple_reference env "
                         "and its MultiDiscrete (5, 10) policy (SimpleReferenceVecEnv, mappo_rollout_episode_reference); pass the flag to run "
                         "the stepwise loop")
+    p.add_argument("--fuse_train_glue", **off,
+                   help="by default a single-process whole-buffer train() runs its once-per-call work in two launches "
+                        "(mappo_train_prologue: advantages, both moment reductions, the ValueNorm updates, the fill of the "
+                        "statistics buffer; mappo_train_epilogue: statistics + after_update); pass the flag to use the separate "
+                        "launches; same results")
     p.add_argument("--dual_update", **off,
                    help="by default the actor's and the critic's fused update run in ONE launch, half the CUs each "
                         "(mappo_actor_critic_update); pass the flag to launch them one after the other")
diff --git a/mappo_amd/csrc/error.hip b/mappo_amd/csrc/error.hip
--- a/mappo_amd/csrc/error.hip
+++ b/mappo_amd/csrc/error.hip
@@ -11,7 +11,7 @@
 }
 
 extern "C" const char *mappo_last_error(void) { return g_err; }
-extern "C" int mappo_abi_version(void) { return 7; }
+extern "C" int mappo_abi_version(void) { return 8; }
 
 ProfSlot g_prof[MAPPO_PROF_COUNT] = {};
 
diff --git a/mappo_amd/csrc/insert.hip b/mappo_amd/csrc/insert.hip
--- a/mappo_amd/csrc/insert.hip
+++ b/mappo_amd/csrc/insert.hip
@@ -133,28 +133,7 @@
   return MAPPO_OK;
 }
 
-#define COPY_MAX 16
-struct CopyBatch {
-  float *dst[COPY_MAX];
-  const float *src[COPY_MAX];
-  int64_t n[COPY_MAX];
-  int count;
-};
-__global__ __launch_bounds__(256) void copy_batch_kernel(CopyBatch c) {
-  for (int j = 0; j < c.count; ++j) {
-    const float *__restrict__ s = c.src[j];
-    float *__restrict__ d = c.dst[j];
-    const int64_t n = c.n[j];
-    if (((((uintptr_t)s) | ((uintptr_t)d)) & 15) == 0) {
-      const int64_t n4 = n >> 2;
-      for (int64_t i = (int64_t)blockIdx.x * blockDim.x + threadIdx.x; i < n4; i += (int64_t)gridDim.x * blockDim.x)
-        reinterpret_cast<float4 *>(d)[i] = reinterpret_cast<const float4 *>(s)[i];
-      for (int64_t i = (n4 << 2) + (int64_t)blockIdx.x * blockDim.x + threadIdx.x; i < n; i += (int64_t)gridDim.x * blockDim.x) d[i] = s[i];
-    } else {
-      for (int64_t i = (int64_t)blockIdx.x * blockDim.x + threadIdx.x; i < n; i += (int64_t)gridDim.x * blockDim.x) d[i] = s[i];
-    }
-  }
-}
+__global__ __launch_bounds__(256) void copy_batch_kernel(CopyBatch c) { copy_batch_body(c, blockIdx.x, gridDim.x); }
 
 extern "C" int mappo_copy_batch(int32_t count, float *const *dst, const float *const *src, const int64_t *n_floats,
                                 mappo_stream_t stream) {
@@ -167,10 +146,7 @@
     c.dst[j] = dst[j]; c.src[j] = src[j]; c.n[j] = n_floats[j];
     total += n_floats[j];
   }
-  int64_t nb = (total / 4 + 255) / 256;
-  if (nb < 1) nb = 1;
-  if (nb > 1024) nb = 1024;
-  hipLaunchKernelGGL(copy_batch_kernel, dim3((unsigned)nb), dim3(256), 0, as_stream(stream), c);
+  hipLaunchKernelGGL(copy_batch_kernel, dim3((unsigned)copy_batch_blocks(total)), dim3(256), 0, as_stream(stream), c);
   MAPPO_CHECK_LAUNCH("copy_batch");
   return MAPPO_OK;
 }
diff --git a/mappo_amd/csrc/insert_core.h b/mappo_amd/csrc/insert_core.h
--- a/mappo_amd/csrc/insert_core.h
+++ b/mappo_amd/csrc/insert_core.h
@@ -121,3 +121,33 @@
     }
   }
 }
+
+
+#define COPY_MAX 16
+struct CopyBatch {
+  float *dst[COPY_MAX];
+  const float *src[COPY_MAX];
+  int64_t n[COPY_MAX];
+  int count;
+};
+static inline int copy_batch_blocks(int64_t total_floats) {
+  int64_t nb = (total_floats / 4 + 255) / 256;
+  if (nb < 1) nb = 1;
+  if (nb > 1024) nb = 1024;
+  return (int)nb;
+}
+__device__ __forceinline__ void copy_batch_body(const CopyBatch &c, int bid, int nb) {
+  for (int j = 0; j < c.count; ++j) {
+    const float *__restrict__ s = c.src[j];
+    float *__restrict__ d = c.dst[j];
+    const int64_t n = c.n[j];
+    if (((((uintptr_t)s) | ((uintptr_t)d)) & 15) == 0) {
+      const int64_t n4 = n >> 2;
+      for (int64_t i = (int64_t)bid * blockDim.x + threadIdx.x; i < n4; i += (int64_t)nb * blockDim.x)
+        reinterpret_cast<float4 *>(d)[i] = reinterpret_cast<const float4 *>(s)[i];
+      for (int64_t i = (n4 << 2) + (int64_t)bid * blockDim.x + threadIdx.x; i < n; i += (int64_t)nb * blockDim.x) d[i] = s[i];
+    } else {
+      for (int64_t i = (int64_t)bid * blockDim.x + threadIdx.x; i < n; i += (int64_t)nb * blockDim.x) d[i] = s[i];
+    }
+  }
+}
diff --git a/mappo_amd/csrc/mlp.hip b/mappo_amd/csrc/mlp.hip
--- a/mappo_amd/csrc/mlp.hip
+++ b/mappo_amd/csrc/mlp.hip
@@ -2,6 +2,7 @@
 #include "mlp_upd.h"
 #include "mlp_upd2.h"
 #include "mlp_upd16.h"
+#include "stats_core.h"
 #include <stdlib.h>
 
 #ifdef MLP_STAMPS
@@ -740,22 +741,7 @@
                                                           int use_value_active, double *__restrict__ stats,
                                                           double *__restrict__ acc) {
   __shared__ double smem[16 * 4];
-  double v[4] = {0.0, 0.0, 0.0, 0.0};
-  for (int b = threadIdx.x; b < na; b += blockDim.x) { v[0] += pa[b * 4 + 0]; v[1] += pa[b * 4 + 1]; v[2] += pa[b * 4 + 2]; }
-  for (int b = threadIdx.x; b < nc; b += blockDim.x) v[3] += pc[b * 4 + 0];
-  block_sum<4>(v, smem);
-  if (threadIdx.x == 0) {
-    const double sa = mb_moments[2] > 0.0 ? mb_moments[2] : 1.0;
-    const double Bg = mb_moments[3] > 0.0 ? mb_moments[3] : 1.0;
-    const double den_pi = use_policy_active ? sa : Bg, den_v = use_value_active ? sa : Bg;
-    stats[0] = v[3] / den_v;
-    stats[1] = -v[0] / den_pi;
-    stats[2] = v[1] / den_pi;
-    stats[3] = v[2] / Bg;
-    stats[4] = mb_moments[2];
-    stats[5] = mb_moments[3];
-    if (acc) { acc[0] += stats[0]; acc[1] += stats[1]; acc[2] += stats[2]; acc[3] += stats[3]; }
-  }
+  update_stats_body(pa, pc, na, nc, mb_moments, use_policy_active, use_value_active, stats, acc, smem);
 }
 
 extern "C" int mappo_update_stats(const double *actor_partials, int32_t n_actor, const double *critic_partials,
diff --git a/mappo_amd/csrc/stats.hip b/mappo_amd/csrc/stats.hip
--- a/mappo_amd/csrc/stats.hip
+++ b/mappo_amd/csrc/stats.hip
@@ -1,27 +1,11 @@
-#include "common.h"
-
-#define STAT_BLOCK 256
-#define STAT_MAX_BLOCKS 1024
-
-static inline int stat_blocks(int64_t n) {
-  int64_t b = (n + STAT_BLOCK * 4 - 1) / (STAT_BLOCK * 4);
-  if (b < 1) b = 1;
-  if (b > STAT_MAX_BLOCKS) b = STAT_MAX_BLOCKS;
-  return (int)b;
-}
+#include "stats_core.h"
 
 template <int NV>
 __global__ __launch_bounds__(STAT_BLOCK) void final_reduce_kernel(const double *__restrict__ partials, int nblk,
                                                                  double *__restrict__ out, double extra) {
   __shared__ double smem[16 * NV];
   double v[NV];
-#pragma unroll
-  for (int i = 0; i < NV; ++i) v[i] = 0.0;
-  for (int b = threadIdx.x; b < nblk; b += blockDim.x) {
-#pragma unroll
-    for (int i = 0; i < NV; ++i) v[i] += partials[(size_t)b * NV + i];
-  }
-  block_sum<NV>(v, smem);
+  final_reduce_sum<NV>(partials, nblk, v, smem);
   if (threadIdx.x == 0) {
 #pragma unroll
     for (int i = 0; i < NV; ++i) out[i] = v[i];
@@ -39,15 +23,8 @@
   const VnStats vn = vn_stats(vn_state);
   double v[3] = {0.0, 0.0, 0.0};
   const int64_t stride = (int64_t)gridDim.x * blockDim.x;
-  for (int64_t i = (int64_t)blockIdx.x * blockDim.x + threadIdx.x; i < n; i += stride) {
-    const float a = returns[i] - (value_preds[i] * vn.sd + vn.mean);
-    adv[i] = a;
-    if (active[i] != 0.f) {
-      v[0] += (double)a;
-      v[1] += (double)a * (double)a;
-      v[2] += 1.0;
-    }
-  }
+  for (int64_t i = (int64_t)blockIdx.x * blockDim.x + threadIdx.x; i < n; i += stride)
+    adv_moments_term(returns[i], value_preds[i], active[i], vn, adv + i, v);
   block_sum<3>(v, smem);
   if (threadIdx.x == 0) {
     partials[blockIdx.x * 3 + 0] = v[0];
@@ -102,10 +79,7 @@
   const int64_t stride = (int64_t)gridDim.x * blockDim.x;
   for (int64_t i = (int64_t)blockIdx.x * blockDim.x + threadIdx.x; i < B; i += stride) {
     const int64_t row = rows ? (int64_t)rows[i] : i;
-    const float r = returns[row];
-    v[0] += (double)r;
-    v[1] += (double)r * (double)r;
-    v[2] += (double)active[row];
+    minibatch_moments_term(returns[row], active[row], v);
   }
   block_sum<3>(v, smem);
   if (threadIdx.x == 0) {
@@ -147,17 +121,7 @@
 }
 
 __global__ void valuenorm_update_n_kernel(float *vn_state, const double *mb_moments, float w, float omw, int n, float *states_out) {
-  const double B = mb_moments[3] > 0.0 ? mb_moments[3] : 1.0;
-  const float bm = (float)(mb_moments[0] / B);
-  const float bsq = (float)(mb_moments[1] / B);
-  float s0 = vn_state[0], s1 = vn_state[1], s2 = vn_state[2];
-  for (int e = 0; e < n; ++e) {
-    s0 = __fadd_rn(__fmul_rn(s0, w), __fmul_rn(bm, omw));
-    s1 = __fadd_rn(__fmul_rn(s1, w), __fmul_rn(bsq, omw));
-    s2 = __fadd_rn(__fmul_rn(s2, w), omw);
-    states_out[3 * e + 0] = s0; states_out[3 * e + 1] = s1; states_out[3 * e + 2] = s2;
-  }
-  vn_state[0] = s0; vn_state[1] = s1; vn_state[2] = s2;
+  valuenorm_update_n_body(vn_state, mb_moments[0], mb_moments[1], mb_moments[3], w, omw, n, states_out);
 }
 
 extern "C" int mappo_valuenorm_update_n(float *vn_state, const double *mb_moments, double beta, int32_t n, float *states_out,
diff --git a/mappo_amd/csrc/stats_core.h b/mappo_amd/csrc/stats_core.h
--- /dev/null
+++ b/mappo_amd/csrc/stats_core.h
@@ -0,0 +1,77 @@
+#pragma once
+#include "common.h"
+
+#define STAT_BLOCK 256
+#define STAT_MAX_BLOCKS 1024
+
+static inline int stat_blocks(int64_t n) {
+  int64_t b = (n + STAT_BLOCK * 4 - 1) / (STAT_BLOCK * 4);
+  if (b < 1) b = 1;
+  if (b > STAT_MAX_BLOCKS) b = STAT_MAX_BLOCKS;
+  return (int)b;
+}
+
+template <int NV>
+__device__ __forceinline__ void final_reduce_sum(const double *partials, int nblk, double (&v)[NV], double *smem ) {
+#pragma unroll
+  for (int i = 0; i < NV; ++i) v[i] = 0.0;
+  for (int b = threadIdx.x; b < nblk; b += blockDim.x) {
+#pragma unroll
+    for (int i = 0; i < NV; ++i) v[i] += partials[(size_t)b * NV + i];
+  }
+  block_sum<NV>(v, smem);
+}
+
+__device__ __forceinline__ void adv_moments_term(float ret, float value_pred, float active, const VnStats &vn, float *adv_i,
+                                                 double (&v)[3]) {
+  const float a = ret - (value_pred * vn.sd + vn.mean);
+  *adv_i = a;
+  if (active != 0.f) {
+    v[0] += (double)a;
+    v[1] += (double)a * (double)a;
+    v[2] += 1.0;
+  }
+}
+
+__device__ __forceinline__ void minibatch_moments_term(float r, float active, double (&v)[3]) {
+  v[0] += (double)r;
+  v[1] += (double)r * (double)r;
+  v[2] += (double)active;
+}
+
+__device__ __forceinline__ void valuenorm_update_n_body(float *vn_state, double m0, double m1, double m3, float w, float omw, int n,
+                                                        float *states_out) {
+  const double B = m3 > 0.0 ? m3 : 1.0;
+  const float bm = (float)(m0 / B);
+  const float bsq = (float)(m1 / B);
+  float s0 = vn_state[0], s1 = vn_state[1], s2 = vn_state[2];
+  for (int e = 0; e < n; ++e) {
+    s0 = __fadd_rn(__fmul_rn(s0, w), __fmul_rn(bm, omw));
+    s1 = __fadd_rn(__fmul_rn(s1, w), __fmul_rn(bsq, omw));
+    s2 = __fadd_rn(__fmul_rn(s2, w), omw);
+    states_out[3 * e + 0] = s0; states_out[3 * e + 1] = s1; states_out[3 * e + 2] = s2;
+  }
+  vn_state[0] = s0; vn_state[1] = s1; vn_state[2] = s2;
+}
+
+__device__ __forceinline__ void update_stats_body(const double *__restrict__ pa, const double *__restrict__ pc, int na, int nc,
+                                                  const double *__restrict__ mb_moments, int use_policy_active,
+                                                  int use_value_active, double *__restrict__ stats, double *__restrict__ acc,
+                                                  double *smem ) {
+  double v[4] = {0.0, 0.0, 0.0, 0.0};
+  for (int b = threadIdx.x; b < na; b += blockDim.x) { v[0] += pa[b * 4 + 0]; v[1] += pa[b * 4 + 1]; v[2] += pa[b * 4 + 2]; }
+  for (int b = threadIdx.x; b < nc; b += blockDim.x) v[3] += pc[b * 4 + 0];
+  block_sum<4>(v, smem);
+  if (threadIdx.x == 0) {
+    const double sa = mb_moments[2] > 0.0 ? mb_moments[2] : 1.0;
+    const double Bg = mb_moments[3] > 0.0 ? mb_moments[3] : 1.0;
+    const double den_pi = use_policy_active ? sa : Bg, den_v = use_value_active ? sa : Bg;
+    stats[0] = v[3] / den_v;
+    stats[1] = -v[0] / den_pi;
+    stats[2] = v[1] / den_pi;
+    stats[3] = v[2] / Bg;
+    stats[4] = mb_moments[2];
+    stats[5] = mb_moments[3];
+    if (acc) { acc[0] += stats[0]; acc[1] += stats[1]; acc[2] += stats[2]; acc[3] += stats[3]; }
+  }
+}
diff --git a/mappo_amd/csrc/train_glue.hip b/mappo_amd/csrc/train_glue.hip
--- /dev/null
+++ b/mappo_amd/csrc/train_glue.hip
@@ -0,0 +1,123 @@
+#include "stats_core.h"
+#include "insert_core.h"
+
+struct PrologueArgs {
+  const float *returns, *value_preds, *active;
+  float *vn_state;
+  float *adv;
+  double *partials;
+  int *ticket;
+  double *adv_moments, *mb_moments;
+  float w, omw;
+  int n_epochs;
+  float *states_out;
+  double *zero;
+  int64_t n_zero, n;
+};
+
+__global__ __launch_bounds__(STAT_BLOCK) void train_prologue_kernel(PrologueArgs p) {
+  __shared__ double smem[16 * 3];
+  __shared__ int s_last;
+  const VnStats vn = vn_stats(p.vn_state);
+  double va[3] = {0.0, 0.0, 0.0}, vm[3] = {0.0, 0.0, 0.0};
+  const int64_t stride = (int64_t)gridDim.x * blockDim.x;
+  for (int64_t i = (int64_t)blockIdx.x * blockDim.x + threadIdx.x; i < p.n; i += stride) {
+    const float r = p.returns[i], act = p.active[i];
+    adv_moments_term(r, p.value_preds[i], act, vn, p.adv + i, va);
+    minibatch_moments_term(r, act, vm);
+  }
+  block_sum<3>(va, smem);
+  block_sum<3>(vm, smem);
+  double *pa = p.partials, *pm = p.partials + (size_t)STAT_MAX_BLOCKS * 3;
+  if (threadIdx.x == 0) {
+#pragma unroll
+    for (int i = 0; i < 3; ++i) {
+      pa[(size_t)blockIdx.x * 3 + i] = va[i];
+      pm[(size_t)blockIdx.x * 3 + i] = vm[i];
+    }
+  }
+  asm volatile("s_waitcnt vmcnt(0)" ::: "memory");
+  __syncthreads();
+  if (threadIdx.x == 0) {
+    __builtin_amdgcn_fence(__ATOMIC_RELEASE, "agent");
+    asm volatile("s_waitcnt vmcnt(0)" ::: "memory");
+    const int t = __hip_atomic_fetch_add(p.ticket, 1, __ATOMIC_RELAXED, __HIP_MEMORY_SCOPE_AGENT);
+    const int last = t == (int)gridDim.x - 1;
+    if (last) {
+      __builtin_amdgcn_fence(__ATOMIC_ACQUIRE, "agent");
+      asm volatile("s_waitcnt vmcnt(0)" ::: "memory");
+    }
+    s_last = last;
+  }
+  __syncthreads();
+  if (!s_last) return;
+
+  const int nblk = (int)gridDim.x;
+  double ra[3], rm[3];
+  final_reduce_sum<3>(pa, nblk, ra, smem);
+  final_reduce_sum<3>(pm, nblk, rm, smem);
+  for (int64_t i = threadIdx.x; i < p.n_zero; i += blockDim.x) p.zero[i] = 0.0;
+  if (threadIdx.x == 0) {
+#pragma unroll
+    for (int i = 0; i < 3; ++i) {
+      p.adv_moments[i] = ra[i];
+      p.mb_moments[i] = rm[i];
+    }
+    const double B = (double)p.n;
+    p.mb_moments[3] = B;
+    if (p.vn_state) valuenorm_update_n_body(p.vn_state, rm[0], rm[1], B, p.w, p.omw, p.n_epochs, p.states_out);
+    __hip_atomic_store(p.ticket, 0, __ATOMIC_RELAXED, __HIP_MEMORY_SCOPE_AGENT);
+  }
+}
+
+extern "C" int64_t mappo_train_prologue_workspace_bytes(int64_t n) { return (int64_t)STAT_MAX_BLOCKS * 6 * sizeof(double); }
+
+extern "C" int mappo_train_prologue(const float *returns, const float *value_preds, const float *active_masks, float *vn_state,
+                                    float *adv, double *adv_moments, double *mb_moments, double beta, int32_t n_epochs,
+                                    float *states_out, double *zero, int64_t n_zero, void *workspace, int32_t *ticket, int64_t n,
+                                    mappo_stream_t stream) {
+  MAPPO_REQUIRE(n > 0 && returns && value_preds && active_masks && adv && adv_moments && mb_moments && workspace && ticket,
+                "train_prologue: bad arguments (n=%lld)", (long long)n);
+  MAPPO_REQUIRE(!vn_state || (states_out && n_epochs >= 1), "train_prologue: a ValueNorm state needs states_out and n_epochs >= 1");
+  MAPPO_REQUIRE(n_zero >= 0 && (n_zero == 0 || zero), "train_prologue: bad fill range (n_zero=%lld)", (long long)n_zero);
+  PrologueArgs p;
+  p.returns = returns; p.value_preds = value_preds; p.active = active_masks; p.vn_state = vn_state; p.adv = adv;
+  p.partials = (double *)workspace; p.ticket = (int *)ticket; p.adv_moments = adv_moments; p.mb_moments = mb_moments;
+  p.w = (float)beta; p.omw = (float)(1.0 - beta); p.n_epochs = (int)n_epochs; p.states_out = states_out;
+  p.zero = zero; p.n_zero = n_zero; p.n = n;
+  hipLaunchKernelGGL(train_prologue_kernel, dim3(stat_blocks(n)), dim3(STAT_BLOCK), 0, as_stream(stream), p);
+  MAPPO_CHECK_LAUNCH("train_prologue");
+  return MAPPO_OK;
+}
+
+__global__ __launch_bounds__(256) void train_epilogue_kernel(const double *__restrict__ pa, const double *__restrict__ pc, int na, int nc,
+                                                            const double *__restrict__ mb_moments, int use_policy_active,
+                                                            int use_value_active, double *__restrict__ stats,
+                                                            double *__restrict__ acc, CopyBatch c) {
+  __shared__ double smem[16 * 4];
+  if (blockIdx.x == 0) {
+    update_stats_body(pa, pc, na, nc, mb_moments, use_policy_active, use_value_active, stats, acc, smem);
+    return;
+  }
+  copy_batch_body(c, (int)blockIdx.x - 1, (int)gridDim.x - 1);
+}
+
+extern "C" int mappo_train_epilogue(const double *actor_partials, int32_t n_actor, const double *critic_partials, int32_t n_critic,
+                                    const double *mb_moments, const mappo_ppo_cfg *cfg, double *stats, double *acc, int32_t count,
+                                    float *const *dst, const float *const *src, const int64_t *n_floats, mappo_stream_t stream) {
+  MAPPO_REQUIRE(critic_partials && mb_moments && cfg && stats && n_critic > 0 && n_actor >= 0, "train_epilogue: bad arguments");
+  MAPPO_REQUIRE(count >= 1 && count <= COPY_MAX && dst && src && n_floats, "train_epilogue: bad copy list (count=%d)", count);
+  CopyBatch c;
+  c.count = count;
+  int64_t total = 0;
+  for (int j = 0; j < count; ++j) {
+    MAPPO_REQUIRE(dst[j] && src[j] && n_floats[j] >= 0, "train_epilogue: copy entry %d", j);
+    c.dst[j] = dst[j]; c.src[j] = src[j]; c.n[j] = n_floats[j];
+    total += n_floats[j];
+  }
+  hipLaunchKernelGGL(train_epilogue_kernel, dim3((unsigned)copy_batch_blocks(total) + 1u), dim3(256), 0, as_stream(stream),
+                     actor_partials, critic_partials, actor_partials ? (int)n_actor : 0, (int)n_critic, mb_moments,
+                     cfg->use_policy_active_masks, cfg->use_value_active_masks, stats, acc, c);
+  MAPPO_CHECK_LAUNCH("train_epilogue");
+  return MAPPO_OK;
+}
diff --git a/mappo_amd/ops.py b/mappo_amd/ops.py
--- a/mappo_amd/ops.py
+++ b/mappo_amd/ops.py
@@ -487,6 +487,38 @@
     _lib.check(rc, "mappo_update_stats")
 
 
+def _copy_lists(pairs):
+    n = len(pairs)
+    for d, s_ in pairs:
+        assert d.is_cuda and s_.is_cuda and d.dtype == torch.float32 and s_.dtype == torch.float32 and d.is_contiguous() \
+            and s_.is_contiguous() and d.numel() == s_.numel()
+    return (n, (C.c_void_p * n)(*[d.data_ptr() for d, _ in pairs]), (C.c_void_p * n)(*[s.data_ptr() for _, s in pairs]),
+            (C.c_int64 * n)(*[d.numel() for d, _ in pairs]))
+
+
+def train_prologue_workspace(n, device):
+    return _ws(_lib.load().mappo_train_prologue_workspace_bytes(int(n)), device), torch.zeros(1, dtype=torch.int32, device=device)
+
+
+def train_prologue(returns, value_preds, active_masks, vn_state, adv, adv_moments, mb_moments, beta, n_epochs, states_out, zero,
+                   workspace, ticket):
+    rc = _lib.load().mappo_train_prologue(_ptr(returns), _ptr(value_preds), _ptr(active_masks), _ptr(vn_state, allow_none=True), _ptr(adv),
+                                          _ptr(adv_moments, torch.float64), _ptr(mb_moments, torch.float64), float(beta), int(n_epochs),
+                                          _ptr(states_out, allow_none=True), _ptr(zero, torch.float64, allow_none=True),
+                                          zero.numel() if zero is not None else 0, _ptr(workspace, torch.uint8),
+                                          _ptr(ticket, torch.int32), adv.numel(), _stream())
+    _lib.check(rc, "mappo_train_prologue")
+
+
+def train_epilogue(actor_partials, n_actor, critic_partials, n_critic, mb_moments, cfg, stats, acc, pairs):
+    n, dst, src, cnt = _copy_lists(pairs)
+    rc = _lib.load().mappo_train_epilogue(_ptr(actor_partials, torch.float64, allow_none=True), int(n_actor),
+                                          _ptr(critic_partials, torch.float64), int(n_critic), _ptr(mb_moments, torch.float64),
+                                          C.byref(cfg), _ptr(stats, torch.float64), _ptr(acc, torch.float64, allow_none=True),
+                                          n, dst, src, cnt, _stream())
+    _lib.check(rc, "mappo_train_epilogue")
+
+
 def mlp_features(params, desc, x, rows, B, featT):
     rc = _lib.load().mappo_mlp_features(_ptr(params), C.byref(desc), _ptr(x), _ptr(rows, torch.int32, allow_none=True), int(B),
                                         _ptr(featT), _stream())
diff --git a/mappo_amd/utils/shared_buffer.py b/mappo_amd/utils/shared_buffer.py
--- a/mappo_amd/utils/shared_buffer.py
+++ b/mappo_amd/utils/shared_buffer.py
@@ -160,9 +160,12 @@
         self.step = (s + 1) % self.episode_length
 
     def after_update(self):
+        ops.copy_batch(self.after_update_pairs())
+
+    def after_update_pairs(self):
         arrs = [a for a in (self.share_obs, self.obs, self.rnn_states, self.rnn_states_critic, self.masks, self.bad_masks,
                             self.active_masks, self.available_actions) if a is not None]
-        ops.copy_batch([(a[0], a[-1]) for a in arrs])
+        return [(a[0], a[-1]) for a in arrs]
 
     def chooseafter_update(self):
         for arr in (self.rnn_states, self.rnn_states_critic, self.masks, self.bad_masks):
```

After: 80.07 million agent-steps/s (median of 6 runs). 1.3% higher.
